# wenet-e2e/wesep

Hardware: AMD Instinct MI355X
Metric: utterances/sec (4 s, 16 kHz, 2-spk) fwd+bwd, pBSRNN (higher is better)
Workload: dtype bf16x3+fp16x2+fp16x1 split products (+fp8 lo terms), fp32 accumulate; 1 GPU; pBSRNN FiLM multi-fuse, 6 repeats, feature_dim 128, fixed 256-d embeddings; fwd + SI-SDR + bwd + per-tensor clip + Adam-L2; bf16x3 (x-projections, projections, d(hcat), BN / mask GEMMs) + fp16x2 (recurrent products of all four recurrence kernels, d(xn)) + fp16x1 (LSTM weight gradients); 2-byte saved gates / d(gates); fp32 accumulate; BPTT kernels: W_hh as fp16 hi + block-scaled FP8 lo; the lo term; rows_per_gpu=32, global_rows=32, samples_per_row=64000, parallelism=dp1

## Files before the change

include/wesep_hip.h:

```cpp
#ifndef WESEP_HIP_H_
#define WESEP_HIP_H_

#ifdef __cplusplus
extern "C" {
#endif

#define WS_ABI_VERSION 20
#define WS_OK 0
#define WS_ERR_INVALID (-1)
#define WS_ERR_LAUNCH (-2)

int ws_abi_version(void);
const char* ws_last_error(void);

#define WS_PROF_LSTM_FWD 0
#define WS_PROF_LSTM_BWD 1
#define WS_PROF_GEMM_NT 2
#define WS_PROF_GEMM_TN 3
#define WS_PROF_NKINDS 4
int ws_prof_enable(int on);
int ws_prof_collect(int kind, double* total_ms, long long* launches);
int ws_debug_dirty_lds(float value, int nblocks, int spins, float* sink, void* stream);
int ws_debug_occupy(int nblocks, int usec, const unsigned* stop, float* sink, void* stream);

// ... 236 lines not shown

typedef struct ws_gemm_b2p_args {
  const float* A;
  const float* Wpack;
  const float* bias;
  const float* R;
  float* C;
  ws_seqmap sm;
  long long ldc;
  int N, K;
  int a_fmt, pad_;
  const unsigned* amax;
  void* a16_out;
} ws_gemm_b2p_args;
int ws_gemm_b2p(const ws_gemm_b2p_args* a, void* stream);

typedef struct ws_gemm_tnb_args {
  const float* G;
  const float* A0;
  const float* A1;
  float* slab;
  float* bslab;
  float* aslab;
  long long slab_stride, bslab_stride, aslab_stride;
  int g_width, g_off, g_cols;
  int a0_width, a0_off, a0_cols, a0_shift;
  int a1_width, a1_off, a1_cols, a1_shift;
  int nblk, L, nsplit, blocks_per_split;
  int g_fmt;
  const unsigned* amax;
  int a_fmt, pad_;
} ws_gemm_tnb_args;
int ws_gemm_tnb(const ws_gemm_tnb_args* a, void* stream);

typedef struct ws_bands {
  const int* band_of_bin;
  const int* band_f0;
  const int* band_bw;
  int nband, nbins;
} ws_bands;
int ws_stft_bandsplit(const float* wav, int R, int T, const ws_bands* b, float* xbs, void* stream);
int ws_stft_bandsplit_len(const float* wav, int R, int T, const int* lengths, const ws_bands* b, float* xbs, void* stream);
int ws_mask_istft_frames(const float* xbs, const float* mask3, int R, int Tf, const ws_bands* b,
                         float* frames, void* stream);
int ws_istft_ola(const float* frames, int R, int Tf, int T, float* wav, void* stream);
int ws_istft_ola_len(const float* frames, int R, int Tf, int T, const int* lengths, float* wav, void* stream);
int ws_mask_istft_bwd(const float* dwav, const float* xbs, const float* mask3, int R, int Tf,
                      int T, const ws_bands* b, float* dmask3, void* stream);

int ws_affine_fwd(const float* z, const float* a, const float* b, float a0, long long rows,
                  int rows_per_r, int N, float* out, void* stream);
int ws_affine_bwd(const float* dz, const float* z_in, const float* a, float a0, long long rows,
                  int rows_per_r, int N, int nsplit, float* dz_in, float* da_slab, float* db_slab,
                  float* da, float* db, unsigned* counter, void* stream);

int ws_sisdr_fwd(const float* est, const float* tgt, int R, int T, float eps, float* rowstat,
                 float* loss, void* stream);
int ws_sisdr_bwd(const float* est, const float* tgt, const float* rowstat, const float* gout,
                 int R, int T, float* dest, void* stream);

typedef struct ws_tensor_ref {
  float* param;
  float* grad;
  float* exp_avg;
  float* exp_avg_sq;
  long long numel;
// ... 233 lines not shown
```

wesep_amd/_lib.py:

```python
import ctypes as C
import os

import numpy as np
import torch

_HERE = os.path.dirname(os.path.abspath(__file__))
LIB_PATH = os.environ.get("WESEP_HIP_LIB") or os.path.join(_HERE, "libwesep_hip.so")

WS_OK = 0
PROF_LSTM_FWD, PROF_LSTM_BWD, PROF_GEMM_NT, PROF_GEMM_TN = 0, 1, 2, 3
LSTM_H = 256
ABI_VERSION = 20
GATES_F32, GATES_H2, GATES_H2S, GATES_H2F = 0, 1, 2, 3
DGATES_EXP = 8


def dgates_scale(amax_bits: int) -> float:
    e = (int(amax_bits) >> 23) & 0xFF
    return 1.0 if e in (0, 255) else 2.0 ** (min(max(DGATES_EXP + 254 - e, 1), 253) - 127)


LSTM_F32_MT1, LSTM_F32_MT2, LSTM_BF16X3, LSTM_BF16X3_BLK, LSTM_BF16X3_BLK16 = 1, 2, 3, 4, 5
LSTM_PACK_FLOATS = 2 * 4 * LSTM_H * LSTM_H

# ... 136 lines not shown
    "ws_pack_w_f16": (_i, [_p, _i, _i, _ll, _i, _i, _p, _p]),
    "ws_pack_w_f16f8": (_i, [_p, _i, _i, _ll, _i, _p, _p]),
    "ws_gemm_nt": (_i, [C.POINTER(GemmNTArgs), _p]),
    "ws_gemm_tn": (_i, [C.POINTER(GemmTNArgs), _p]),
    "ws_reduce_slabs": (_i, [_p, _i, _ll, _ll, _p, _i, _ll, _p]),
    "ws_transpose": (_i, [_p, _i, _i, _ll, _p, _p]),
    "ws_group_stats": (_i, [_p, C.POINTER(GroupsGeom), _f, _p, _p]),
    "ws_group_stats_len": (_i, [_p, C.POINTER(GroupsGeom), _p, _i, _f, _p, _p]),
    "ws_gn_bwd_reduce": (_i, [_p, _p, _p, _p, _p, C.POINTER(GroupsGeom), _p, _p]),
    "ws_gn_bwd_apply": (_i, [_p, _p, _p, _p, _p, _p, _p, C.POINTER(GroupsGeom), _p, _p]),
    "ws_gn_param_grad": (_i, [_p, _p, _p, C.POINTER(GroupsGeom), _i, _p, _p]),
    "ws_gn_bwd_fused": (_i, [_p, _p, _p, _p, _p, C.POINTER(GroupsGeom), _i, _p, _p, _p, _p, _p]),
    "ws_gn_bwd_fused2": (_i, [_p, _p, _p, _p, _p, _p, C.POINTER(GroupsGeom), _i, _p, _p, _p, _p, _p]),
    "ws_gn_bwd_apply_pg": (_i, [_p, _p, _p, _p, _p, _p, C.POINTER(GroupsGeom), _p, _p, _p, _p, _p]),
    "ws_lstm_pack": (_i, [_p, _p, _p, _p, _i, _p]),
    "ws_lstm_fwd": (_i, [C.POINTER(LstmArgs), _p]),
    "ws_lstm_bwd": (_i, [C.POINTER(LstmArgs), _p]),
    "ws_lstm_fwd_cluster": (_i, [C.POINTER(LstmClusterArgs), _p]),
    "ws_lstm_bwd_cluster": (_i, [C.POINTER(LstmClusterArgs), _p]),
    "ws_lstm_fwd_cluster2": (_i, [C.POINTER(LstmCluster2Args), _p]),
    "ws_lstm_pack_pair": (_i, [_p, _p, _p, _p]),
    "ws_lstm_pack_pair_f16": (_i, [_p, _p, _p, _p]),
    "ws_lstm_pack_pair_f8": (_i, [_p, _p, _p, _p]),
    "ws_lstm_pack_pair_f8mx": (_i, [_p, _p, _p, _p]),
    "ws_lstm_pack_bwd_f8": (_i, [_p, _p, _p, _p]),
    "ws_lstm_pack_dx_f8": (_i, [_p, _p, _p]),
    "ws_lstm_bwd_pair": (_i, [C.POINTER(LstmPairArgs), _p]),
    "ws_lstm_cat_ih": (_i, [_p, _p, _p, _p, _p, _p, _i, _p, _p, _p]),
    "ws_pack_w": (_i, [_p, _i, _i, _ll, _i, _i, _p, _p]),
    "ws_gemm_p2b": (_i, [C.POINTER(GemmP2BArgs), _p]),
    "ws_gemm_p2b_len": (_i, [C.POINTER(GemmP2BArgs), _p, _i, _p]),
    "ws_gemm_b2p": (_i, [C.POINTER(GemmB2PArgs), _p]),
    "ws_gemm_tnb": (_i, [C.POINTER(GemmTNBArgs), _p]),
    "ws_stft_bandsplit": (_i, [_p, _i, _i, C.POINTER(Bands), _p, _p]),
    "ws_stft_bandsplit_len": (_i, [_p, _i, _i, _p, C.POINTER(Bands), _p, _p]),
    "ws_mask_istft_frames": (_i, [_p, _p, _i, _i, C.POINTER(Bands), _p, _p]),
    "ws_istft_ola": (_i, [_p, _i, _i, _i, _p, _p]),
    "ws_istft_ola_len": (_i, [_p, _i, _i, _i, _p, _p, _p]),
    "ws_mask_istft_bwd": (_i, [_p, _p, _p, _i, _i, _i, C.POINTER(Bands), _p, _p]),
    "ws_affine_fwd": (_i, [_p, _p, _p, _f, _ll, _i, _i, _p, _p]),
    "ws_affine_bwd": (_i, [_p, _p, _p, _f, _ll, _i, _i, _i, _p, _p, _p, _p, _p, _p, _p]),
    "ws_sisdr_fwd": (_i, [_p, _p, _i, _i, _f, _p, _p, _p]),
    "ws_sisdr_bwd": (_i, [_p, _p, _p, _p, _i, _i, _p, _p]),
    "ws_flat_stats": (_i, [_p, _i, _ll, C.c_float, _i, _p, _p, _p]),
    "ws_prelu_fwd": (_i, [_p, _p, _p, _ll, _i, _i, _p, _p]),
    "ws_prelu_bwd": (_i, [_p, _p, _p, _ll, _p, _p, _i, _p]),
    "ws_dwconv_fwd": (_i, [_p, _p, _p, _p, _p, _p, _i, _i, _i, _i, _i, _i, _p, _p]),
    "ws_dwconv_bwd": (_i, [_p, _p, _p, _p, _p, _p, _i, _i, _i, _i, _i, _i, _p, _i, _i, _p, _p]),
    "ws_dwconv_ex_fwd": (_i, [_p, _p, _p, _p, _p, _p, _i, _i, _i, _i, _i, _i, _i, _p, _p]),
    "ws_dwconv_ex_bwd": (_i, [_p, _p, _p, _p, _p, _p, _i, _i, _i, _i, _i, _i, _i, _p, _i, _i, _p, _p]),
    "ws_chan_sums": (_i, [_p, _p, _p, _i, _i, _i, _i, _i, _p, _p]),
    "ws_norm_ab": (_i, [_p, _p, _i, _i, _ll, _p, _p]),
    "ws_norm_bwd_apply_cl": (_i, [_p, _p, _p, _p, _p, _p, _ll, _i, _i, _p, _p]),
    "ws_maskmul_fwd": (_i, [_p, _ll, _p, _ll, _i, _p, _p]),
    "ws_maskmul_bwd": (_i, [_p, _p, _ll, _p, _ll, _i, _p, _ll, _p, _p]),
    "ws_relu_mask": (_i, [_p, _p, _ll, _p]),
    "ws_ola_fwd": (_i, [_p, _p, _i, _i, _i, _i, _i, _p, _p]),
    "ws_ola_bwd": (_i, [_p, _i, _i, _i, _i, _i, _p, _p]),
    "ws_sum_partial": (_i, [_p, _ll, _p, _i, _p]),
    "ws_bn_stats": (_i, [_p, _ll, _i, C.c_float, C.c_float, _p, _p, _i, _p, _p, _p]),
    "ws_bn_prelu_fwd": (_i, [_p, _p, _p, _p, _p, _p, _ll, _i, _p, _p, _p]),
    "ws_bn_bwd": (_i, [_p, _p, _p, _p, _ll, _i, _i, _p, _p, _p, _p]),
    "ws_maxpool3_fwd": (_i, [_p, _i, _i, _i, _p, _p]),
    "ws_maxpool3_bwd": (_i, [_p, _p, _i, _i, _i, _p, _p]),
    "ws_bcast_rows": (_i, [_p, C.c_float, _i, _ll, _i, _p, _p]),
    "ws_cross_entropy": (_i, [_p, _p, _i, _i, _p, _p, _p]),
# ... 123 lines not shown
```

wesep_amd/blstm_core.py:

```python
import math
import os
from typing import NamedTuple

import numpy as np
import torch

from . import _lib as L
from . import dev

H = L.LSTM_H
G4 = 4 * H
N = 128


def _empty(dev_, *shape):
    return torch.empty(*shape, device=dev_, dtype=torch.float32)


def _reduce_new(slab, nsplit, stride, shape):
    out = _empty(slab.device, *shape)
    dev.reduce_slabs(slab, nsplit, stride, int(np.prod(shape)), out)
    return out


# ... 1 lines not shown
    return int(os.environ.get("WESEP_H2_PROBE", "0"))


_PROBE_SAT = [0, 0.0]


def _probe_round(t, kind, packed=False):
    if kind == "f16":
        t.copy_(t.half().float())
    elif kind == "u16":
        v = t.view(-1, 2, 4, 64 * 128)
        v[:, :, 2].mul_(0.5).add_(0.5)
        v.copy_(torch.floor(v * 65535.0 + 0.5) / 65535.0)
        v[:, :, 2].mul_(2.0).sub_(1.0)
    elif packed and torch.cuda.is_available():
        t.view(torch.int32).bitwise_and_(-65536)
    else:
        t.copy_(t.bfloat16().float())


def tnb_a16() -> bool:
    return os.environ.get("WESEP_TNB_A16", "1") != "0"


def pair_rfmt(gfmt) -> int:
    rf = int(os.environ.get("WESEP_PAIR_RF", "3"))
    if rf not in (0, 1, 2, 3):
        raise ValueError(f"WESEP_PAIR_RF={rf}: 0, 1, 2 or 3")
    return rf if gfmt == L.GATES_H2F else 0


def dxn_fmt(g_fmt) -> int:
    return 3 if g_fmt == 2 and os.environ.get("WESEP_DXN_F8", "1") != "0" else g_fmt


def band_rfmt(gfmt, lmode) -> int:
    rf = int(os.environ.get("WESEP_BAND_RF", "3"))
    if rf not in (0, 2, 3):
        raise ValueError(f"WESEP_BAND_RF={rf}: 0, 2 or 3")
    if rf == 3 and os.environ.get("WESEP_BAND_DX", "0") == "1":
        rf = 2
    return rf if gfmt == L.GATES_H2F and lmode == L.LSTM_BF16X3_BLK else 0


def band_dx(brf, seq, geo) -> bool:
    return (brf == 2 and os.environ.get("WESEP_BAND_DX", "0") == "1" and not seq.nvalid and dev.gn_bwd_fused_ok(geo))


_SIDE_STREAMS = {}


def _side_stream(device):
    key = (device.type, device.index)
    if key not in _SIDE_STREAMS:
        pr = os.environ.get("WESEP_SIDE_PRIORITY")
        _SIDE_STREAMS[key] = torch.cuda.Stream(device=device, priority=int(pr)) if pr else torch.cuda.Stream(device=device)
    return _SIDE_STREAMS[key]


_PENDING = {}


def _pending(device):
    return _PENDING.setdefault((device.type, device.index), [])


# ... 206 lines not shown
            dev.lstm_pack(*W("whh"), pack_f, pack_b, lmode)
            return pack_f, pack_b
        if kind == "hh8":
            pack = _empty(d, L.LSTM_PACK_FLOATS)
            dev.lstm_pack_bwd_f8(*W("whh"), pack)
            return pack
        if kind == "wx8":
            pack = _empty(d, L.LSTM_DX_PACK_FLOATS)
            dev.lstm_pack_dx_f8(W("cat")[0], pack)
            return pack
        if kind in ("hhp", "hhp16"):
            pack = _empty(d, L.LSTM_PACK_FLOATS)
            dev.lstm_pack_pair(*W("whh"), pack, f16=pair_rf if kind == "hhp16" else 0)
            return pack
        if kind in ("fused", "fused16", "fused8"):
            fpack = _empty(d, L.LSTM_FUSED_PACK_FLOATS)
            dev.lstm_pack_fused(wih_f.contiguous(), wih_r.contiguous(), *W("whh"), fpack,
                                hfmt={"fused": 0, "fused16": 1, "fused8": 5}[kind])
            return fpack
        if kind == "wih":
            out = _empty(d, 2 * G4 * N)
            dev.pack_w(W("cat")[0], 2 * G4, N, N, out, order=0)
            return out
        if kind in ("wihT", "wihT16", "wihT8"):
            out = _empty(d, N * 2 * G4)
            dev.pack_w(W("cat")[0], N, 2 * G4, N, out, trans=True, order=1, f16={"wihT": 0, "wihT16": 1, "wihT8": 2}[kind])
            return out
        if kind == "pw":
            return proj_w.contiguous()
        if kind == "proj":
            out = _empty(d, N * 2 * H)
            dev.pack_w(W("pw"), N, 2 * H, 2 * H, out, order=1)
            return out
        if kind == "projT":
            out = _empty(d, 2 * H * N)
            dev.pack_w(W("pw"), 2 * H, N, 2 * H, out, trans=True, order=0)
            return out
        raise KeyError(kind)


class BlstmPlan(NamedTuple):
    nb: int
    lmode: int
    cluster: bool
    fwd: str
    bptt: str
    grad: bool
    gfmt: int
    g_fmt: int
    a16: bool
    pair_rfmt: int
    band_rfmt: int
    band_dx: bool
    a_fmt: int


_WIHT_KIND = {0: "wihT", 1: "wihT", 2: "wihT16", 3: "wihT8"}


def make_plan(seq, device, grad, gn_geo=None, ragged=False) -> BlstmPlan:
    lmode = dev.lstm_blk_mode(seq.nseq)
    cluster = dev.lstm_cluster_ok(seq, device)
    bptt = _bptt_kind(seq, device, cluster)
    gfmt = L.GATES_F32 if bptt == "cluster" else dev.gates_fmt()
    h2 = gfmt != L.GATES_F32
    if ragged:
        fwd = "cluster" if cluster else "stream"
    elif dev.lstm_fuse_ok(seq.nseq, cluster):
        fwd = "fused"
    elif cluster:
        fwd = "cluster2" if h2 and dev.lstm_cluster2_on() else "cluster"
    else:
        fwd = "stream"
    g_fmt = {L.GATES_H2: 1, L.GATES_H2F: 2}.get(gfmt, 0)
    brf = band_rfmt(gfmt, lmode) if grad and bptt == "stream" else 0
    return BlstmPlan(
        nb=dev.bl_num_blocks(seq), lmode=lmode, cluster=cluster, fwd=fwd, bptt=bptt, grad=grad, gfmt=gfmt, g_fmt=g_fmt,
        a16=gfmt == L.GATES_H2F and grad and tnb_a16(), pair_rfmt=pair_rfmt(gfmt) if grad and bptt == "pair" else 0,
        band_rfmt=brf, band_dx=bool(brf) and gn_geo is not None and band_dx(brf, seq, gn_geo), a_fmt=dxn_fmt(g_fmt))


def consume_once(ctx, who):
    if ctx.consumed:
        raise L.WesepHipError(f"{who}: second backward through the same graph (retain_graph / multi-loss loops): "
                              "the blocked path consumes its saved gates in place; run the forward again")
    ctx.consumed = True


def blstm_forward(plan, W, x, seq, res, bias, norm=None, steps=None):
    d = x.device
    norm = norm or {}
    if steps is not None and (plan.fwd in ("fused", "cluster2") or plan.grad):
        raise L.WesepHipError(f"blstm_forward: per-sequence step counts with forward branch '{plan.fwd}', grad={plan.grad}: "
                              "only the branches over precomputed gates know them, and only the forward")
    lens = dict(steps=steps[0], steps_div=steps[1]) if steps is not None else {}
    nb, gfmt, lmode = plan.nb, plan.gfmt, plan.lmode
    h2 = gfmt != L.GATES_F32
    wcat, bcat = W("cat")
    whf, whr = W("whh")
    xn = _empty(d, nb, 32 * N)
    cbuf, hcat = _empty(d, nb, 32 * 2 * H), _empty(d, nb, 32 * 2 * H)
    gates = _empty(d, dev.blh_floats(nb, 2 * G4)) if h2 else _empty(d, nb, 32 * 2 * G4)
    xn16 = _empty(d, dev.blh_floats(nb, N)) if plan.a16 else None
    hcat16 = _empty(d, dev.blh_floats(nb, 2 * H)) if plan.a16 else None
    if plan.fwd == "fused":
        dev.gemm_p2b(A=x, lda=N, sm=seq, Wpack=None, N=0, C_out=None, A_bl=xn, A_bl16=xn16, **norm)
        hf = dev.lstm_fused_hfmt(gfmt)
        dev.lstm_fwd_fused(gates, cbuf, hcat, xn, W("fused8" if hf & 4 else "fused16" if hf else "fused"), bcat, seq, gfmt=gfmt,
                           hfmt=hf)
    elif plan.fwd == "cluster2":
        dev.gemm_p2b(A=x, lda=N, sm=seq, Wpack=None, N=0, C_out=None, A_bl=xn, A_bl16=xn16, **norm)
        tw = dev.lstm_fwd_cluster2(gates, cbuf, hcat, xn, wcat, bcat, whf, whr, seq, dbg=_cluster_dbg())
        pre = dev.fallback_scratch(d, nb * 32 * 2 * G4)
        dev.gemm_p2b(A=x, lda=N, sm=seq, Wpack=W("wih"), N=2 * G4, C_out=pre, bias=bcat, run_if=tw, **norm)
        dev.lstm_fwd(gates, cbuf, hcat, W("hh")[0], seq, lmode, run_if=tw, gfmt=gfmt, gates_in=pre)
        del pre
    else:
        pre = _empty(d, nb, 32 * 2 * G4) if h2 else gates
        xproj = dict(A=x, lda=N, sm=seq, Wpack=W("wih"), N=2 * G4, C_out=pre, bias=bcat, A_bl=xn, A_bl16=xn16, **norm, **lens)
        rec = dict(gfmt=gfmt, gates_in=pre) if h2 else {}
        dev.gemm_p2b(**xproj)
        if _h2_probe() & 768 and not torch.cuda.is_available():
            pre.copy_(pre.half().float() if _h2_probe() & 256 else pre.bfloat16().float())
        if plan.fwd == "cluster":
            tw = dev.lstm_fwd_cluster(gates, cbuf, hcat, whf, whr, seq, dbg=_cluster_dbg(), **rec)
            if not h2:
                dev.gemm_p2b(run_if=tw, **xproj)
            dev.lstm_fwd(gates, cbuf, hcat, W("hh")[0], seq, lmode, run_if=tw, **rec)
        else:
            dev.lstm_fwd(gates, cbuf, hcat, W("hh")[0], seq, lmode, **rec)
        del pre
    out = torch.empty_like(res)
    dev.gemm_b2p(A=hcat, K=2 * H, sm=seq, Wpack=W("proj"), C_out=out, ldc=N, bias=bias, R=res, a16_out=hcat16)
    if _h2_probe() and not h2:
        if _h2_probe() & 1:
            _probe_round(gates, "f16")
        if _h2_probe() & 8:
            _probe_round(gates, "u16")
        if _h2_probe() & 4:
            _probe_round(cbuf, "f16")
    if plan.grad:
        W("projT")
        if not plan.band_dx:
            W(_WIHT_KIND[plan.a_fmt])
        if plan.bptt == "pair":
            W("hhp16" if plan.pair_rfmt else "hhp")
        if (plan.bptt == "stream" and not plan.band_rfmt) or (plan.bptt == "pair" and h2):
            W("hh")
        if plan.bptt == "stream" and plan.band_rfmt:
            W("hh8")
            if plan.band_dx:
                W("wx8")
    return out, (gates, cbuf, hcat, xn16 if plan.a16 else xn, hcat16)


def blstm_bptt(plan, W, gates, cbuf, hcat, dout, seq, release):
    d = dout.device
    nb, gfmt = plan.nb, plan.gfmt
    dh, dout_bl = _empty(d, nb, 32 * 2 * H), _empty(d, nb, 32 * N)
    dxn2 = None
    amax = amax_word(d) if gfmt == L.GATES_H2F else None
    dev.gemm_p2b(A=dout, lda=N, sm=seq, Wpack=W("projT"), N=2 * H, C_out=dh, A_bl=dout_bl, amax=amax)
    if _h2_probe() & 16:
        _probe_round(dh, "bf16")
    ready = mark_wgrads_ready(d) if release else None
    if plan.bptt == "cluster":
        dg = gates
        dev.lstm_bwd_cluster(gates, cbuf, dh, *W("whh"), seq)
    elif gfmt == L.GATES_F32:
        dg = gates
        if plan.bptt == "pair":
            dev.lstm_bwd_pair(gates, cbuf, dh, W("hhp"), seq, dbg=_pair_dbg())
        else:
            dev.lstm_bwd(gates, cbuf, hcat, dh, W("hh")[1], seq, plan.lmode)
    elif plan.bptt == "pair":
        dg = _empty(d, nb, 32 * 2 * G4) if gfmt == L.GATES_H2S else _empty(d, dev.blh_floats(nb, 2 * G4))
        rf = plan.pair_rfmt
        tw = dev.lstm_bwd_pair(gates, cbuf, dh, W("hhp16" if rf else "hhp"), seq, gfmt=gfmt, dgates=dg, repairable=True,
                               dbg=_pair_dbg(), amax=amax, rfmt=rf, dbg_buf=_pair_stamp_buf(d, seq.L))
        dev.lstm_bwd(gates, cbuf, hcat, dh, W("hh")[1], seq, plan.lmode, gfmt=gfmt, dgates=dg, run_if=tw, amax=amax)
    else:
        dg = _empty(d, nb, 32 * 2 * G4) if gfmt == L.GATES_H2S else gates
        brf = plan.band_rfmt
        if plan.band_dx:
            dxn2 = _empty(d, 2, dout.numel() // N, N)
        dev.lstm_bwd(gates, cbuf, hcat, dh, W("hh8") if brf else W("hh")[1], seq, plan.lmode, gfmt=gfmt,
                     dgates=dg if gfmt == L.GATES_H2S else None, amax=amax, rfmt=brf, dxn=dxn2,
                     wxpack=W("wx8") if dxn2 is not None else None)
    if _h2_probe() & 2 and gfmt == L.GATES_F32:
        _probe_round(gates, "bf16", packed=True)
    if _h2_probe() & 32 and gfmt == L.GATES_F32 and not torch.cuda.is_available():
        amax = float(dh.abs().max())
        S = 2.0 ** (10 - math.floor(math.log2(amax))) if amax > 0 and math.isfinite(amax) else 1.0
        sc = gates * S
        _PROBE_SAT[0] += int((sc.abs() > 65504.0).sum())
        _PROBE_SAT[1] = max(_PROBE_SAT[1], float(sc.abs().max()) / 65504.0)
        gates.copy_(sc.clamp(-65504.0, 65504.0).half().float() / S)
    if ready is not None:
        flush_deferred_wgrads(d, ready)
    return dg, dout_bl, amax, dxn2


def weight_grads(gates, xn, hcat, dout_bl, seq, nb, g_fmt=0, amax=None, hcat16=None):
    d = gates.device
    a_fmt = 1 if hcat16 is not None else 0
    if _h2_probe() & 192 and not torch.cuda.is_available() and not a_fmt:
        rnd = (lambda t: t.half().float()) if _h2_probe() & 64 else (lambda t: t.bfloat16().float())
        xn, hcat = rnd(xn), rnd(hcat)
    if os.environ.get("WESEP_PROBE_SKIP_WGRAD") == "1":
        z_ = lambda *s_: torch.zeros(*s_, device=d)
        return [z_(G4, N), z_(G4, H), z_(G4), z_(G4), z_(G4, N), z_(G4, H), z_(G4), z_(G4), z_(N, 2 * H), z_(N)]
    if _h2_probe() & 1024 and not torch.cuda.is_available() and amax is not None:
        S = L.dgates_scale(int(amax.reshape(-1)[0]))
        hcat = hcat.half().float()
        dout_bl = (dout_bl * S).half().float() / S
    ns, bps = dev.tnb_splits(nb, (2 * H) // 128)
    slab, aslab = _empty(d, ns, 2 * H * N), _empty(d, ns, N)
    dev.gemm_tnb(G=hcat, g_width=2 * H, g_off=0, g_cols=2 * H, A0=dout_bl, a0_width=N, a0_off=0, a0_cols=N,
                 nblk=nb, L_=seq.L, slab=slab, nsplit=ns, blocks_per_split=bps, aslab=aslab)
    dproj_w = _reduce_new(slab, ns, 2 * H * N, (2 * H, N)).t().contiguous()
    dproj_b = _reduce_new(aslab, ns, N, (N,))
    ns, bps = dev.tnb_splits(nb, G4 // 128)
    slab, bslab = _empty(d, ns, G4 * (N + H)), _empty(d, ns, G4)
    dwih, dwhh, db = [], [], []
    for di in (0, 1):
        dev.gemm_tnb(G=gates, g_width=2 * G4, g_off=di * G4, g_cols=G4, A0=xn, a0_width=N, a0_off=0,
                     a0_cols=N, A1=hcat16 if a_fmt else hcat, a1_width=2 * H, a1_off=di * H, a1_cols=H,
                     a1_shift=(-1 if di == 0 else 1), nblk=nb, L_=seq.L, slab=slab, nsplit=ns,
                     blocks_per_split=bps, bslab=bslab, g_fmt=g_fmt, amax=amax, a_fmt=a_fmt)
        dw = _reduce_new(slab, ns, G4 * (N + H), (G4, N + H))
        dwih.append(dw[:, :N].contiguous())
        dwhh.append(dw[:, N:].contiguous())
        db.append(_reduce_new(bslab, ns, G4, (G4,)))
    return [dwih[0], dwhh[0], db[0], db[0].clone(), dwih[1], dwhh[1], db[1], db[1].clone(),
            dproj_w, dproj_b]


def blstm_weight_grads(plan, dg, xn, hcat, dout_bl, amax, hcat16, seq, box, order=tuple(range(10))):
    if box is None:
        wg = weight_grads(dg, xn, hcat, dout_bl, seq, plan.nb, plan.g_fmt, amax, hcat16)
        return [wg[i] for i in order]
    prod = torch.cuda.current_stream()

    def job(side):
        wg = weight_grads(dg, xn, hcat, dout_bl, seq, plan.nb, plan.g_fmt, amax, hcat16)
        box.grads = [wg[i] for i in order]
        box.event = torch.cuda.Event()
        box.event.record(side)
        keep_for_side(box, (dg, xn, hcat, dout_bl, amax, hcat16), side, prod)
    defer_wgrad(dg.device, job)
    return [None] * len(order)


def blstm_dxn(plan, W, dg, amax, dxn2, seq, rows):
    if dxn2 is not None:
        return dxn2[0], dxn2[1]
    dxn = _empty(dg.device, rows, N)
    dev.gemm_b2p(A=dg, K=2 * G4, sm=seq, Wpack=W(_WIHT_KIND[plan.a_fmt]), C_out=dxn, ldc=N, a_fmt=plan.a_fmt, amax=amax)
    return dxn, None
```

wesep_amd/csrc/gemm_blk.hip:

```cpp
#include <stdlib.h>

#include <type_traits>

#include "common.h"

typedef __bf16 bf16x8 __attribute__((ext_vector_type(8)));
typedef unsigned int u32x4 __attribute__((ext_vector_type(4)));
typedef unsigned int u32x2 __attribute__((ext_vector_type(2)));
typedef float f32x2 __attribute__((ext_vector_type(2)));
typedef _Float16 f16x8 __attribute__((ext_vector_type(8)));
typedef _Float16 f16x2 __attribute__((ext_vector_type(2)));
typedef int i32x4 __attribute__((ext_vector_type(4)));
typedef int v8i __attribute__((ext_vector_type(8)));
typedef __fp16 h16x2 __attribute__((ext_vector_type(2)));

__device__ __forceinline__ f32x16 mfma32(bf16x8 a, bf16x8 b, f32x16 c) {
  return __builtin_amdgcn_mfma_f32_32x32x16_bf16(a, b, c, 0, 0, 0);
}

__device__ __forceinline__ void split8(const float* v, bf16x8& hi, bf16x8& lo) {
#pragma unroll
  for (int j = 0; j < 8; ++j) {
    hi[j] = (__bf16)v[j];
    lo[j] = (__bf16)(v[j] - (float)hi[j]);
// ... 485 lines not shown
      if (off[k] >= 0) *reinterpret_cast<f32x4*>(p.C + off[k]) = v[k];
    __syncthreads();
  }
}

extern "C" int ws_gemm_b2p(const ws_gemm_b2p_args* a, void* stream) {
  WS_REQUIRE(a && a->A && a->Wpack && a->C, "ws_gemm_b2p: null pointer");
  WS_REQUIRE(a->N == 128, "ws_gemm_b2p: N must be 128 (got %d)", a->N);
  WS_REQUIRE(a->a_fmt >= 0 && a->a_fmt <= 3 && (a->a_fmt < 2 || a->amax), "ws_gemm_b2p: a_fmt %d (2 / 3 need amax)", a->a_fmt);
  WS_REQUIRE(a->a_fmt == 0 || !a->a16_out, "ws_gemm_b2p: a16_out goes with a_fmt 0 (got a_fmt %d)", a->a_fmt);
  WS_REQUIRE(a->K > 0 && a->K % 64 == 0, "ws_gemm_b2p: K %% 64 (K=%d)", a->K);
  WS_REQUIRE(a->ldc >= a->N && a->ldc % 4 == 0, "ws_gemm_b2p: ldc >= N and ldc %% 4 == 0 (16-byte row pieces)");
  WS_REQUIRE(a->sm.nseq > 0 && a->sm.L > 0 && a->sm.sq_div > 0, "ws_gemm_b2p: bad sequence map");
  const int nblk = ((a->sm.nseq + 31) / 32) * a->sm.L;
  hipStream_t s = (hipStream_t)stream;
  ws_prof_begin(WS_PROF_GEMM_NT, s);
  if (a->a_fmt == 3)
    hipLaunchKernelGGL(gemm_b2p_kernel<3>, dim3((nblk + 7) / 8), dim3(512), 0, s, *a);
  else if (a->a_fmt == 2)
    hipLaunchKernelGGL(gemm_b2p_kernel<2>, dim3((nblk + 7) / 8), dim3(512), 0, s, *a);
  else if (a->a_fmt == 1)
    hipLaunchKernelGGL(gemm_b2p_kernel<1>, dim3((nblk + 7) / 8), dim3(512), 0, s, *a);
  else
    hipLaunchKernelGGL(gemm_b2p_kernel<0>, dim3((nblk + 7) / 8), dim3(512), 0, s, *a);
  ws_prof_end(WS_PROF_GEMM_NT, s);
  return ws_check_launch("ws_gemm_b2p");
}

typedef __bf16 bf16x4 __attribute__((ext_vector_type(4)));
#define TB_LD 40

typedef __bf16 bf16x2 __attribute__((ext_vector_type(2)));

template <int TA, bool ASUM>
__global__ __launch_bounds__(512, 2) void gemm_tnb_kernel(const ws_gemm_tnb_args p) {
  constexpr int NCOL = 128 * (1 + TA);
  constexpr int PLANE = NCOL * TB_LD;
  constexpr int NG = (1 + TA) / 2;
  constexpr int TN = TA == 1 ? 1 : TA;
  __shared__ __attribute__((aligned(16))) __bf16 ldsA[2 * PLANE];
  __shared__ __attribute__((aligned(16))) __bf16 ldsB[2 * PLANE];
  const int tid = threadIdx.x, lane = tid & 63, l31 = lane & 31, half = lane >> 5;
  const int w = __builtin_amdgcn_readfirstlane(tid >> 6);
  const int wm = w >> 2, wn = w & 3;
  const int gt = blockIdx.y, split = blockIdx.x;
  const int L = p.L;
  const int b_begin = split * p.blocks_per_split;
  const int b_end = min(p.nblk, b_begin + p.blocks_per_split);

  const float* gbase[NG];
  long long gstride[NG];
  int gshift[NG], gcol[NG];
#pragma unroll
  for (int r = 0; r < NG; ++r) {
    const int g = tid + 512 * r;
    const int part = g >> 8, quad = (g >> 3) & 31, sg = g & 7;
    gcol[r] = part * 128 + 4 * quad;
    if (part == 0) {
      gbase[r] = p.G + (long long)((p.g_off + gt * 128) / 4 + quad) * 128 + sg * 16;
      gstride[r] = 32LL * p.g_width;
      gshift[r] = 0;
    } else {
      const int c0 = (part - 1) * 128;
      const bool s1 = c0 >= p.a0_cols;
      const float* base = s1 ? p.A1 : p.A0;
      const int off = s1 ? p.a1_off + c0 - p.a0_cols : p.a0_off + c0;
      gbase[r] = base + (long long)(off / 4 + quad) * 128 + sg * 16;
      gstride[r] = 32LL * (s1 ? p.a1_width : p.a0_width);
      gshift[r] = s1 ? p.a1_shift : p.a0_shift;
    }
  }
  const int sg = tid & 7;

  f32x4 rq[2][NG][4];
  bool use[2][NG];
  auto load_block = [&](int b, int slot) {
    const int tile = b / L, step = b - tile * L;
#pragma unroll
    for (int r = 0; r < NG; ++r) {
      const int sa = step + gshift[r];
      use[slot][r] = sa >= 0 && sa < L;
      const float* src = gbase[r] + (long long)(use[slot][r] ? b + gshift[r] : b) * gstride[r];
#pragma unroll
      for (int j = 0; j < 4; ++j) rq[slot][r][j] = *reinterpret_cast<const f32x4*>(src + 4 * j);
    }
  };
  float csum[NG][4];
#pragma unroll
  for (int r = 0; r < NG; ++r)
#pragma unroll
    for (int c = 0; c < 4; ++c) csum[r][c] = 0.f;
  auto store_piece = [&](int slot, __bf16* lds, unsigned live, int pc) {
    const int r = pc >> 2, c = pc & 3;
    unsigned e[4];
#pragma unroll
    for (int j = 0; j < 4; ++j) {
      const float f = rq[slot][r][j][c];
      e[j] = __float_as_uint(f);
    }
    if (r > 0) {
      const unsigned m = use[slot][r] ? 0xffffffffu : 0u;
#pragma unroll
      for (int j = 0; j < 4; ++j) e[j] &= m;
    }
    if (r == 0 || ASUM) {
      const bf16x2 ones = __builtin_bit_cast(bf16x2, live);
#pragma unroll
      for (int j = 0; j < 4; ++j)
        csum[r][c] = __builtin_amdgcn_fdot2_f32_bf16(__builtin_bit_cast(bf16x2, e[j]), ones, csum[r][c], false);
    }
    uint2 hi, lo;
    hi.x = __builtin_amdgcn_perm(e[1], e[0], WS_SEL_HI16);
    hi.y = __builtin_amdgcn_perm(e[3], e[2], WS_SEL_HI16);
    lo.x = __builtin_amdgcn_perm(e[1], e[0], WS_SEL_LO16);
    lo.y = __builtin_amdgcn_perm(e[3], e[2], WS_SEL_LO16);
    const int o = (gcol[r] + c) * TB_LD + 4 * sg;
    *reinterpret_cast<uint2*>(lds + o) = hi;
    *reinterpret_cast<uint2*>(lds + PLANE + o) = lo;
  };
  auto store_block = [&](int slot, __bf16* lds, unsigned live) {
#pragma unroll
    for (int pc = 0; pc < 4 * NG; ++pc) store_piece(slot, lds, live, pc);
  };

  f32x16 acc[2][TN];
#pragma unroll
  for (int e = 0; e < 2; ++e)
#pragma unroll
    for (int f = 0; f < TN; ++f)
#pragma unroll
      for (int r = 0; r < 16; ++r) acc[e][f][r] = 0.f;
// ... 351 lines not shown
    for (int f = 0; f < TN; ++f) {
      const int ac_ = wn * 32 * TN + f * 32 + l31;
      if (ac_ < ncols) {
#pragma unroll
        for (int r = 0; r < 16; ++r) {
          const int grow = gt * 128 + wm * 64 + e * 32 + (r & 3) + 8 * (r >> 2) + 4 * half;
          out[(long long)grow * ncols + ac_] = GFMT >= 2 ? acc[e][f][r] * inv_out : acc[e][f][r];
        }
      }
    }
#pragma unroll
  for (int c = 0; c < 4; ++c) {
    float t = gsum[c];
    t += __shfl_xor(t, 1, 64);
    t += __shfl_xor(t, 2, 64);
    t += __shfl_xor(t, 4, 64);
    t += __shfl_xor(t, 8, 64);
    if (p.bslab && sp == 0) p.bslab[(long long)split * p.bslab_stride + gt * 128 + 4 * qg + c] = GFMT >= 2 ? t * inv_s : t;
  }
  if (ASUM && gt == 0 && p.aslab) {
#pragma unroll
    for (int r = 0; r < 2; ++r)
#pragma unroll
      for (int c = 0; c < 4; ++c) {
        float t = asum[r][c];
        t += __shfl_xor(t, 1, 64);
        t += __shfl_xor(t, 2, 64);
        t += __shfl_xor(t, 4, 64);
        if (r == 1) t += __shfl_xor(t, 8, 64);
        const bool first = r == 0 ? (tid & 7) == 0 : (tid & 15) == 0;
        if (first) p.aslab[(long long)split * p.aslab_stride + acol[r] - 128 + c] = t;
      }
  }
}

extern "C" int ws_gemm_tnb(const ws_gemm_tnb_args* a, void* stream) {
  WS_REQUIRE(a && a->G && a->A0 && a->slab, "ws_gemm_tnb: null pointer");
  WS_REQUIRE(a->g_cols > 0 && a->g_cols % 128 == 0 && a->g_off % 4 == 0 && a->g_width % 4 == 0,
             "ws_gemm_tnb: G column range");
  WS_REQUIRE(a->a0_cols > 0 && a->a0_cols % 128 == 0 && a->a0_off % 4 == 0 && a->a0_width % 4 == 0,
             "ws_gemm_tnb: A0 column range");
  WS_REQUIRE(a->a1_cols == 0 || (a->A1 && a->a1_cols % 128 == 0 && a->a1_off % 4 == 0 && a->a1_width % 4 == 0),
             "ws_gemm_tnb: A1 column range");
  const int ta = (a->a0_cols + a->a1_cols) / 128;
  WS_REQUIRE(ta == 1 || ta == 3, "ws_gemm_tnb: A columns must total 128 or 384 (got %d)", ta * 128);
  WS_REQUIRE(a->a0_shift == 0, "ws_gemm_tnb: only A1 can be shifted (a0_shift = %d)", a->a0_shift);
  WS_REQUIRE(a->g_fmt == 0 || ((a->g_fmt == 1 || a->g_fmt == 2) && ta == 3),
             "ws_gemm_tnb: g_fmt 1 / 2 (2-byte G) are built for 384 A columns");
  WS_REQUIRE(a->g_fmt != 2 || a->amax, "ws_gemm_tnb: g_fmt = 2 (scaled fp16 G) needs amax");
  WS_REQUIRE(a->a_fmt == 0 || (a->a_fmt == 1 && a->g_fmt == 2 && !a->aslab && ta == 3),
             "ws_gemm_tnb: a_fmt = 1 (fp16 A operands) is built for g_fmt = 2, 384 A columns, no aslab");
  WS_REQUIRE(a->nblk > 0 && a->L > 0 && a->nblk % a->L == 0 && a->nsplit > 0 && a->blocks_per_split > 0 &&
                 (long long)a->nsplit * a->blocks_per_split >= a->nblk,
             "ws_gemm_tnb: bad block split");
  hipStream_t s = (hipStream_t)stream;
  dim3 grid(a->nsplit, a->g_cols / 128), block(512);
  ws_prof_begin(WS_PROF_GEMM_TN, s);
  static const int gdepth = [] { const char* e = getenv("WS_TNB_GDEPTH"); return e && atoi(e) == 2 ? 2 : 4; }();
  const char* f16env = getenv("WS_TNB_F16");
  const bool f16mm = !(f16env && atoi(f16env) == 0);
  if (a->a_fmt == 1)
    hipLaunchKernelGGL((gemm_tnb16_kernel<false, 3, 4, 1>), grid, block, 0, s, *a);
  else if (a->g_fmt == 2 && f16mm && a->aslab)
    hipLaunchKernelGGL((gemm_tnb16_kernel<true, 3, 4>), grid, block, 0, s, *a);
  else if (a->g_fmt == 2 && f16mm)
    hipLaunchKernelGGL((gemm_tnb16_kernel<false, 3, 4>), grid, block, 0, s, *a);
// ... 22 lines not shown
```

wesep_amd/csrc/lstm.hip:

```cpp
#include "common.h"

#define LH WS_LSTM_H
#define LG (4 * LH)
#define HL_LD 68
#define DG_LD 260

__device__ __forceinline__ f32x4 mfma16(float a, float b, f32x4 c) {
  return __builtin_amdgcn_mfma_f32_16x16x4f32(a, b, c, 0, 0, 0);
}

__device__ __forceinline__ float fast_sigmoid(float x) {
  return __builtin_amdgcn_rcpf(1.f + __expf(-x));
}
__device__ __forceinline__ float fast_tanh(float x) {
  const float ax = fabsf(x);
  const float e = __expf(-2.f * ax);
  const float t = (1.f - e) * __builtin_amdgcn_rcpf(1.f + e);
  return copysignf(t, x);
}

__global__ void lstm_pack_kernel(const float* __restrict__ whh_f, const float* __restrict__ whh_r,
                                 float* __restrict__ pf, float* __restrict__ pb) {
  const int total = 2 * LG * LH;
  for (int idx = blockIdx.x * blockDim.x + threadIdx.x; idx < total; idx += gridDim.x * blockDim.x) {
// ... 316 lines not shown
      f32x4 a[MT];
#pragma unroll
      for (int mt = 0; mt < MT; ++mt)
        a[mt] = *reinterpret_cast<const f32x4*>(arow + mt * (64 * DG_LD) + 4 * ks4);
#pragma unroll
      for (int q = 0; q < 4; ++q)
#pragma unroll
        for (int s = 0; s < 2; ++s)
#pragma unroll
          for (int mt = 0; mt < MT; ++mt) dh[mt][s] = mfma16(a[mt][q], bcur[s][q], dh[mt][s]);
      bcur[0] = bnxt[0];
      bcur[1] = bnxt[1];
    }
    __syncthreads();
  }
}

static int lstm_check(const ws_lstm_args* a, bool bwd, const char* who) {
  WS_REQUIRE(a && a->gates && a->cbuf && a->hcat && a->wpack, "%s: null pointer", who);
  WS_REQUIRE(!bwd || a->dhcat, "%s: null dhcat", who);
  WS_REQUIRE(a->nseq > 0 && a->L > 0 && a->sq_div > 0, "%s: bad nseq/L/sq_div", who);
  WS_REQUIRE((a->mode & 255) >= WS_LSTM_F32_MT1 && (a->mode & 255) <= WS_LSTM_BF16X3_BLK16, "%s: bad mode %d", who,
             a->mode);
  WS_REQUIRE(!a->run_if || (!bwd && (a->mode & 255) >= WS_LSTM_BF16X3) || (bwd && (a->mode & 255) >= WS_LSTM_BF16X3_BLK),
             "%s: run_if is honoured by the split-bf16 forward kernels and the blocked-layout BPTT kernels only", who);
  WS_REQUIRE(a->gfmt >= WS_GATES_F32 && a->gfmt <= WS_GATES_H2F, "%s: bad gfmt %d", who, a->gfmt);
  WS_REQUIRE(a->gfmt != WS_GATES_H2F || !bwd || a->amax, "%s: WS_GATES_H2F needs amax", who);
  WS_REQUIRE(a->gfmt == WS_GATES_F32 || (a->mode & 255) >= WS_LSTM_BF16X3_BLK,
             "%s: gfmt %d is a format of the blocked-layout modes", who, a->gfmt);
  WS_REQUIRE(a->gfmt == WS_GATES_F32 || bwd || a->gates_in, "%s: gfmt %d needs gates_in (the fp32 pre-activations)", who,
             a->gfmt);
  WS_REQUIRE(a->gfmt != WS_GATES_H2S || !bwd || a->dgates, "%s: WS_GATES_H2S needs dgates", who);
  WS_REQUIRE(a->gfmt == WS_GATES_F32 || ((a->mode >> 8) & 7) == 0, "%s: probe builds are WS_GATES_F32 only", who);
  WS_REQUIRE(a->rfmt == 0 || ((a->rfmt == 2 || a->rfmt == 3) && bwd && a->mode == WS_LSTM_BF16X3_BLK && a->gfmt == WS_GATES_H2F),
             "%s: rfmt %d (2 / 3 = fp16 recurrence on fp16 + FP8 weights, 3: the lo term on the FP8 MFMA: ws_lstm_bwd, "
             "WS_LSTM_BF16X3_BLK, WS_GATES_H2F only)", who, a->rfmt);
  WS_REQUIRE(!a->dxn || (bwd && a->rfmt == 2 && a->wxpack && a->dxn_dir_stride > 0 && a->dxn_dir_stride < (1ll << 29) && !a->run_if),
             "%s: dxn (d(xn) inside the BPTT, ABI v19) needs rfmt 2, wxpack (ws_lstm_pack_dx_f8), 0 < dxn_dir_stride < 2^29 floats "
             "(32-bit store offsets) and no run_if", who);
  return WS_OK;
}

extern "C" int ws_lstm_fwd(const ws_lstm_args* a, void* stream) {
  int rc = lstm_check(a, false, "ws_lstm_fwd");
  if (rc != WS_OK) return rc;
  hipStream_t s = (hipStream_t)stream;
  const int per = 16 * a->mode;
  dim3 grid((a->nseq + per - 1) / per, 2), block(512);
  const bool timed = a->run_if == nullptr;
  if (timed) ws_prof_begin(WS_PROF_LSTM_FWD, s);
  if ((a->mode & 255) == WS_LSTM_BF16X3_BLK16)
    ws_launch_lstm_fwd_s16(a, s);
  else if ((a->mode & 255) >= WS_LSTM_BF16X3)
    ws_launch_lstm_fwd_bf16(a, s);
  else if (a->mode == WS_LSTM_F32_MT1)
    hipLaunchKernelGGL((lstm_fwd_kernel<1>), grid, block, 0, s, *a);
  else
    hipLaunchKernelGGL((lstm_fwd_kernel<2>), grid, block, 0, s, *a);
  if (timed) ws_prof_end(WS_PROF_LSTM_FWD, s);
  return ws_check_launch("ws_lstm_fwd");
}

extern "C" int ws_lstm_bwd(const ws_lstm_args* a, void* stream) {
  int rc = lstm_check(a, true, "ws_lstm_bwd");
  if (rc != WS_OK) return rc;
  hipStream_t s = (hipStream_t)stream;
  const int per = 16 * a->mode;
  dim3 grid((a->nseq + per - 1) / per, 2), block(512);
  const bool timed = a->run_if == nullptr;
// ... 13 lines not shown
```

wesep_amd/csrc/lstm_bf16.hip:

```cpp
#include <stdlib.h>

#include "lstm_bf16_common.h"

__global__ void lstm_pack_bf16_kernel(const float* __restrict__ whh_f, const float* __restrict__ whh_r,
                                      __bf16* __restrict__ pf, __bf16* __restrict__ pb) {
  const int total = 2 * LG * LH;
  for (int idx = blockIdx.x * blockDim.x + threadIdx.x; idx < total; idx += gridDim.x * blockDim.x) {
    {
      int r = idx;
      const int j = r & 7; r >>= 3;
      const int lane = r & 63; r >>= 6;
      const int g = r & 3; r >>= 2;
      const int ks = r & 15; r >>= 4;
      const int w = r & 7; r >>= 3;
      const int d = r;
      const float* W = d ? whh_r : whh_f;
      const int row = g * 256 + 32 * w + (lane & 31);
      const int k = 16 * ks + 8 * (lane >> 5) + j;
      const float v = W[row * LH + k];
      const __bf16 hi = (__bf16)v;
      const long long unit = ((((long long)(d * 8 + w) * 16 + ks) * 4 + g) * 2) * 64 + lane;
      pf[unit * 8 + j] = hi;
      pf[(unit + 64) * 8 + j] = (__bf16)(v - (float)hi);
    }
// ... 82 lines not shown
    v0[i] = 256.f * W[row * 128 + u];
    v1[i] = 256.f * W[(row + 1) * 128 + u];
    m = fmaxf(m, fmaxf(fabsf(v0[i]), fabsf(v1[i])));
  }
#pragma unroll
  for (int o = 32; o > 0; o >>= 1) m = fmaxf(m, __shfl_xor(m, o));
  if ((tid & 63) == 0) red[tid >> 6] = m;
  __syncthreads();
  m = red[0];
#pragma unroll
  for (int i = 1; i < 8; ++i) m = fmaxf(m, red[i]);
  const int eb = (int)((__builtin_bit_cast(unsigned, m) >> 23) & 0xffu);
  const float S = (eb > 19 && eb < 255) ? __builtin_bit_cast(float, (unsigned)(eb - 19) << 23) : 1.f;
  char* ob = px + (long long)(d * 8 + w) * WS_DX_REGION;
  if (tid == 0) reinterpret_cast<float*>(ob + 48 * 1024)[grp] = S;
#pragma unroll
  for (int i = 0; i < 2; ++i) {
    const int pi = tid + 512 * i, j2 = pi & 3, lane = (pi >> 2) & 63, f = pi >> 8;
    const _Float16 h0 = (_Float16)v0[i], h1 = (_Float16)v1[i];
    typedef _Float16 f16x2 __attribute__((ext_vector_type(2)));
    typedef short s16x2 __attribute__((ext_vector_type(2)));
    char* cb = ob + (2 * grp + (f >> 1)) * 3072;
    *reinterpret_cast<f16x2*>(cb + (f & 1) * 1024 + lane * 16 + j2 * 4) = f16x2{h0, h1};
    const s16x2 c = __builtin_amdgcn_cvt_scalef32_pk_fp8_f32(s16x2{0, 0}, v0[i] - (float)h0, v1[i] - (float)h1, S, false);
    *reinterpret_cast<short*>(cb + 2048 + (f & 1) * 512 + lane * 8 + j2 * 2) = c[0];
  }
}

int ws_launch_lstm_pack_dx_f8(const float* wcat, float* pack, hipStream_t s) {
  hipLaunchKernelGGL(lstm_pack_dx_f8_kernel, dim3(128), dim3(512), 0, s, wcat, reinterpret_cast<char*>(pack));
  return 0;
}

template <bool BLK, int DBG, int GF = 0>
__global__ __launch_bounds__(512, 2) void lstm_fwd_bf16_kernel(const ws_lstm_args p) {
  __shared__ __attribute__((aligned(16))) __bf16 hl[2][2][SQ * HROW];
  __shared__ __attribute__((aligned(16))) float cl[SQ * (LH + 4)];
  if (p.run_if && *p.run_if == 0u) return;
  const int d = blockIdx.y;
  const int tid = threadIdx.x, lane = tid & 63, l31 = lane & 31, half = lane >> 5;
  const int w = __builtin_amdgcn_readfirstlane(tid >> 6);
  const int L = p.L;

  {
    uint32_t* z = reinterpret_cast<uint32_t*>(&hl[0][0][0]);
    for (int i = tid; i < 2 * SQ * HROW / 2; i += 512) z[i] = 0u;
  }
  const int ss = min((int)blockIdx.x * SQ + l31, p.nseq - 1);
  const long long rowbase =
      BLK ? 0 : (long long)(ss / p.sq_div) * p.sq_s1 + (long long)(ss % p.sq_div) * p.sq_s2;
  const int ubase = 32 * w + 4 * half;
  const int glane = ((d * 256 + 8 * w + half) * 32 + l31) * 16;
  const int clane = ((d * 64 + 8 * w + half) * 32 + l31) * 16;
  auto goff = [&](int t, int g, int j) -> long long {
    return ((rowbase + (long long)t * p.step_rows) * 2 + d) * LG + g * 256 + ubase + 8 * j;
  };
  auto coff = [&](int t, int j) -> long long {
    return (rowbase + (long long)t * p.step_rows) * (2 * LH) + d * LH + ubase + 8 * j;
  };
  const float* gsrc = GF ? p.gates_in : p.gates;
  auto grs = [&](int t) { return mkrsrc(gsrc + (long long)(blockIdx.x * L + t) * (SQ * 2 * LG), SQ * 2 * LG * 4); };
  auto hrs = [&](int t) { return mkrsrc(p.gates + (long long)(blockIdx.x * L + t) * (SQ * LG), SQ * 2 * LG * 2); };
  auto crs = [&](float* b, int t) { return mkrsrc(b + (long long)(blockIdx.x * L + t) * (SQ * 2 * LH), SQ * 2 * LH * 4); };
  auto ld_gate = [&](int t, int g, int j) -> f32x4 {
    if constexpr (BLK) return bld(grs(t), glane, (g * 64 + 2 * j) * 512);
    else return *reinterpret_cast<const f32x4*>(p.gates + goff(t, g, j));
  };
  auto st_gate = [&](const f32x4& v, int t, int g, int j) {
    if constexpr (GF != 0) bst8(g == 2 ? enc_u16x4<true>(v) : enc_u16x4<false>(v), hrs(t), glane >> 1, (g * 64 + 2 * j) * 256);
    else if constexpr (BLK) bst(v, grs(t), glane, (g * 64 + 2 * j) * 512);
    else *reinterpret_cast<f32x4*>(p.gates + goff(t, g, j)) = v;
  };
  auto st_ch = [&](const f32x4& v, float* b, int t, int j) {
    if constexpr (BLK) bst(v, crs(b, t), clane, 2 * j * 512);
    else *reinterpret_cast<f32x4*>(b + coff(t, j)) = v;
  };

  float* cme = &cl[l31 * (LH + 4) + ubase];
#pragma unroll
  for (int j = 0; j < 4; ++j) *reinterpret_cast<f32x4*>(cme + 8 * j) = f32x4{0.f, 0.f, 0.f, 0.f};

  const __amdgpu_buffer_rsrc_t wrs = __builtin_amdgcn_make_buffer_rsrc(
      const_cast<float*>(p.wpack) + (long long)(d * 8 + w) * (16 * 8 * 64 * 4), 0, 16 * 8 * 1024, 0x00020000);
  const int wlane = lane * 16;
  bf16x8 wr[2][8];
#pragma unroll
  for (int s = 0; s < 2; ++s)
#pragma unroll
    for (int f = 0; f < 8; ++f) wr[s][f] = wload(wrs, wlane + (f & 3) * 1024, s * 8192 + (f >> 2) * 4096);

  f32x4 xg[4][4];
  {
    const int t0 = d == 0 ? 0 : L - 1;
#pragma unroll
    for (int gi = 0; gi < 4; ++gi)
#pragma unroll
      for (int j = 0; j < 4; ++j) xg[gi][j] = ld_gate(t0, gi, j);
  }
  __syncthreads();

  for (int step = 0; step < L; ++step) {
    const int t = d == 0 ? step : L - 1 - step;
    const int cur = step & 1;
    int zo = 0;
    asm volatile("" : "+s"(zo));
    const __bf16* hhi = &hl[cur][0][l31 * HROW + 8 * half];
    const __bf16* hlo = &hl[cur][1][l31 * HROW + 8 * half];
    f32x16 acc[4];
#pragma unroll
// ... 43 lines not shown
    for (int j = 0; j < 4; ++j) {
      f32x4 pre[4];
#pragma unroll
      for (int g = 0; g < 4; ++g)
#pragma unroll
        for (int r = 0; r < 4; ++r) pre[g][r] = acc[g][4 * j + r];
      f32x4 vi, vf, vg, vo, vc, vh;
      const f32x4 cold = *reinterpret_cast<const f32x4*>(cme + 8 * j);
#pragma unroll
      for (int r = 0; r < 4; ++r) {
        const float ig = fsig(pre[0][r]);
        const float fg = fsig(pre[1][r]);
        const float gg = ftanh(pre[2][r]);
        const float og = fsig(pre[3][r]);
        const float cn = fg * cold[r] + ig * gg;
        vi[r] = ig;
        vf[r] = fg;
        vg[r] = gg;
        vo[r] = og;
        vc[r] = cn;
        vh[r] = og * ftanh(cn);
      }
      bf16x4 h_hi, h_lo;
      split4(vh, h_hi, h_lo);
      *reinterpret_cast<bf16x4*>(nhi + 8 * j) = h_hi;
      *reinterpret_cast<bf16x4*>(nlo + 8 * j) = h_lo;
      *reinterpret_cast<f32x4*>(cme + 8 * j) = vc;
      if (!(DBG & 1) || step == L - 1) {
        st_gate(vi, t, 0, j);
        st_gate(vf, t, 1, j);
        st_gate(vg, t, 2, j);
        st_gate(vo, t, 3, j);
        st_ch(vc, p.cbuf, t, j);
        if constexpr (BLK) st_ch(pack_hl4(h_hi, h_lo), p.hcat, t, j);
        else st_ch(vh, p.hcat, t, j);
      }
      __builtin_amdgcn_sched_barrier(0);
    }
    __syncthreads();
  }
}

template <bool BLK, int DBG, int GF = 0, int RF = 0, bool DX = false>
__global__ __launch_bounds__(512, 2) void lstm_bwd_bf16_kernel(const ws_lstm_args p) {
  static_assert(RF == 0 || (BLK && GF == WS_GATES_H2F), "the fp16 recurrence takes the scaled-fp16 d(gates) of WS_GATES_H2F");
  static_assert(!DX || RF == 2, "d(xn) in the BPTT rides on the fp16 d(gates) image of rfmt 2");
  __shared__ __attribute__((aligned(16))) __bf16 dgl[RF ? 1 : 2][SQ * DROW];
  __shared__ __attribute__((aligned(16))) f32x4 xred[DX ? 8 * 2 * 64 : 1];
  if (p.run_if && *p.run_if == 0u) return;
  const int d = blockIdx.y, bx = blockIdx.x;
  const int tid = threadIdx.x, lane = tid & 63, l31 = lane & 31, half = lane >> 5;
  const int w = __builtin_amdgcn_readfirstlane(tid >> 6);
  const int L = p.L;
  const int ss = min(bx * SQ + l31, p.nseq - 1);
  const long long rowbase =
      BLK ? 0 : (long long)(ss / p.sq_div) * p.sq_s1 + (long long)(ss % p.sq_div) * p.sq_s2;
  const int ubase = 32 * w + 4 * half;
  const int glane = ((d * 256 + 8 * w + half) * 32 + l31) * 16;
  const int clane = ((d * 64 + 8 * w + half) * 32 + l31) * 16;
  auto goff = [&](int t, int g, int j) -> long long {
    return ((rowbase + (long long)t * p.step_rows) * 2 + d) * LG + g * 256 + ubase + 8 * j;
  };
  auto coff = [&](int t, int j) -> long long {
    return (rowbase + (long long)t * p.step_rows) * (2 * LH) + d * LH + ubase + 8 * j;
  };
  float* gdst = GF == WS_GATES_H2S ? p.dgates : p.gates;
  auto grs = [&](int t) { return mkrsrc(gdst + (long long)(bx * L + t) * (SQ * 2 * LG), SQ * 2 * LG * 4); };
  auto hrs = [&](int t) { return mkrsrc(p.gates + (long long)(bx * L + t) * (SQ * LG), SQ * 2 * LG * 2); };
// ... 269 lines not shown
    if constexpr (DX) {
      const float us = (1.f / 256.f) / dS;
      const unsigned trow = (unsigned)t * (unsigned)p.step_rows * 512u;
#pragma unroll
      for (int i = 0; i < 2; ++i) {
        const f32x4 o = xred[((w ^ 4) * 2 + i) * 64 + lane];
        __builtin_amdgcn_raw_buffer_store_b128(__builtin_bit_cast(u32x4, (keep[i] + o) * us), xors, xoff + trow + 32 * i, 0, 0);
      }
    }
  }
}

#define WS_DBG_DISPATCH(KERNEL)                                                          \
  if ((a->mode & 255) == WS_LSTM_BF16X3_BLK && a->gfmt == WS_GATES_H2) {                 \
    hipLaunchKernelGGL((KERNEL<true, 0, WS_GATES_H2>), grid, block, 0, s, *a);           \
  } else if ((a->mode & 255) == WS_LSTM_BF16X3_BLK && a->gfmt == WS_GATES_H2S) {         \
    hipLaunchKernelGGL((KERNEL<true, 0, WS_GATES_H2S>), grid, block, 0, s, *a);          \
  } else if ((a->mode & 255) == WS_LSTM_BF16X3_BLK && a->gfmt == WS_GATES_H2F) {         \
    hipLaunchKernelGGL((KERNEL<true, 0, WS_GATES_H2F>), grid, block, 0, s, *a);          \
  } else if ((a->mode & 255) == WS_LSTM_BF16X3_BLK) {                                    \
    switch ((a->mode >> 8) & 7) {                                                        \
      case 0: hipLaunchKernelGGL((KERNEL<true, 0>), grid, block, 0, s, *a); break;       \
      case 1: hipLaunchKernelGGL((KERNEL<true, 1>), grid, block, 0, s, *a); break;       \
      case 2: hipLaunchKernelGGL((KERNEL<true, 2>), grid, block, 0, s, *a); break;       \
      case 4: hipLaunchKernelGGL((KERNEL<true, 4>), grid, block, 0, s, *a); break;       \
      default: hipLaunchKernelGGL((KERNEL<true, 7>), grid, block, 0, s, *a); break;      \
    }                                                                                    \
  } else {                                                                               \
    hipLaunchKernelGGL((KERNEL<false, 0>), grid, block, 0, s, *a);                       \
  }

int ws_launch_lstm_fwd_bf16(const ws_lstm_args* a, hipStream_t s) {
  dim3 grid((a->nseq + SQ - 1) / SQ, 2), block(512);
  WS_DBG_DISPATCH(lstm_fwd_bf16_kernel)
  return 0;
}

int ws_launch_lstm_bwd_bf16(const ws_lstm_args* a, hipStream_t s) {
  dim3 grid((a->nseq + SQ - 1) / SQ, 2), block(512);
  if (a->rfmt == 2 && a->dxn) {
    hipLaunchKernelGGL((lstm_bwd_bf16_kernel<true, 0, WS_GATES_H2F, 2, true>), grid, block, 0, s, *a);
    return 0;
  }
  if (a->rfmt == 2) {
    hipLaunchKernelGGL((lstm_bwd_bf16_kernel<true, 0, WS_GATES_H2F, 2>), grid, block, 0, s, *a);
    return 0;
  }
  if (a->rfmt == 3) {
    hipLaunchKernelGGL((lstm_bwd_bf16_kernel<true, 0, WS_GATES_H2F, 3>), grid, block, 0, s, *a);
    return 0;
  }
  WS_DBG_DISPATCH(lstm_bwd_bf16_kernel)
  return 0;
}
```

wesep_amd/csrc/lstm_bf16_common.h:

```cpp
#pragma once
#include "common.h"

typedef __bf16 bf16x8 __attribute__((ext_vector_type(8)));
typedef __bf16 bf16x4 __attribute__((ext_vector_type(4)));

#define LH WS_LSTM_H
#define LG (4 * LH)
#define SQ 32
#define HROW 264
#define DROW 1032

typedef unsigned int u32x4 __attribute__((ext_vector_type(4)));

__device__ __forceinline__ bf16x8 wload(__amdgpu_buffer_rsrc_t rsrc, int voff, int soff) {
  return __builtin_bit_cast(bf16x8, __builtin_amdgcn_raw_buffer_load_b128(rsrc, voff, soff, 0));
}

__device__ __forceinline__ __amdgpu_buffer_rsrc_t mkrsrc(const float* base, unsigned bytes) {
  return __builtin_amdgcn_make_buffer_rsrc(const_cast<float*>(base), 0, bytes, 0x00020000);
}
#ifndef WS_STREAM_AUX
#define WS_STREAM_AUX 2
#endif
__device__ __forceinline__ f32x4 bld(__amdgpu_buffer_rsrc_t r, int voff, int soff) {
// ... 65 lines not shown

__device__ __forceinline__ u32x2 bld8(__amdgpu_buffer_rsrc_t r, int voff, int soff) {
  return __builtin_bit_cast(u32x2, __builtin_amdgcn_raw_buffer_load_b64(r, voff, soff, WS_STREAM_AUX));
}
__device__ __forceinline__ void bst8(const u32x2& v, __amdgpu_buffer_rsrc_t r, int voff, int soff) {
  __builtin_amdgcn_raw_buffer_store_b64(v, r, voff + soff, 0, WS_STREAM_AUX);
}
template <bool TANH>
__device__ __forceinline__ u32x2 enc_u16x4(const f32x4& v) {
  const float s = TANH ? WS_U16_TANH : WS_U16_SIG, o = TANH ? WS_U16_TANH + 0.5f : 0.5f;
  unsigned u[4];
#pragma unroll
  for (int j = 0; j < 4; ++j) u[j] = (unsigned)__builtin_fmaf(v[j], s, o);
  return u32x2{u[0] | (u[1] << 16), u[2] | (u[3] << 16)};
}
template <bool TANH>
__device__ __forceinline__ f32x4 dec_u16x4(const u32x2& c) {
  const float s = TANH ? 1.f / WS_U16_TANH : 1.f / WS_U16_SIG, o = TANH ? -1.f : 0.f;
  f32x4 v;
  v[0] = __builtin_fmaf((float)(c[0] & 0xffffu), s, o);
  v[1] = __builtin_fmaf((float)(c[0] >> 16), s, o);
  v[2] = __builtin_fmaf((float)(c[1] & 0xffffu), s, o);
  v[3] = __builtin_fmaf((float)(c[1] >> 16), s, o);
  return v;
}
__device__ __forceinline__ u32x2 bf16x4_bits(const bf16x4& v) { return __builtin_bit_cast(u32x2, v); }
typedef _Float16 f16x4 __attribute__((ext_vector_type(4)));
__device__ __forceinline__ u32x2 enc_f16x4(const f32x4& vs) {
  f16x4 h;
#pragma unroll
  for (int j = 0; j < 4; ++j) h[j] = (_Float16)vs[j];
  return __builtin_bit_cast(u32x2, h);
}
template <int GF>
__device__ __forceinline__ u32x2 enc_dgates(const f32x4& v, const bf16x4& hi) {
  if constexpr (GF == WS_GATES_H2F) return enc_f16x4(v);
  else return bf16x4_bits(hi);
}
template <int GF>
__device__ __forceinline__ float dh_in(float dh, float rec, float S) {
  if constexpr (GF == WS_GATES_H2F) return __builtin_fmaf(dh, S, rec);
  else return dh + rec;
}

template <int GF> struct gate_cell { typedef f32x4 type; };
template <> struct gate_cell<WS_GATES_H2> { typedef u32x2 type; };
template <> struct gate_cell<WS_GATES_H2S> { typedef u32x2 type; };
template <> struct gate_cell<WS_GATES_H2F> { typedef u32x2 type; };
template <bool TANH> __device__ __forceinline__ f32x4 gate_val(const f32x4& c) { return c; }
template <bool TANH> __device__ __forceinline__ f32x4 gate_val(const u32x2& c) { return dec_u16x4<TANH>(c); }
```

wesep_amd/csrc/lstm_bf16_s16.hip:

```cpp
#include "lstm_bf16_common.h"

#define S16 16

__device__ __forceinline__ f32x4 mfma16(bf16x8 a, bf16x8 b, f32x4 c) {
  return __builtin_amdgcn_mfma_f32_16x16x32_bf16(a, b, c, 0, 0, 0);
}

__global__ void lstm_pack_s16_kernel(const float* __restrict__ whh_f, const float* __restrict__ whh_r,
                                     __bf16* __restrict__ pf, __bf16* __restrict__ pb) {
  const int total = 2 * LG * LH;
  for (int idx = blockIdx.x * blockDim.x + threadIdx.x; idx < total; idx += gridDim.x * blockDim.x) {
    {
      int r = idx;
      const int j = r & 7; r >>= 3;
      const int lane = r & 63; r >>= 6;
      const int tile = r & 7; r >>= 3;
      const int ks = r & 7; r >>= 3;
      const int w = r & 7; r >>= 3;
      const int d = r;
      const float* W = d ? whh_r : whh_f;
      const int row = (tile >> 1) * 256 + 32 * w + 16 * (tile & 1) + (lane & 15);
      const int k = 32 * ks + 8 * (lane >> 4) + j;
      const float v = W[row * LH + k];
      const __bf16 hi = (__bf16)v;
      const long long unit = ((((long long)(d * 8 + w) * 8 + ks) * 8 + tile) * 2) * 64 + lane;
      pf[unit * 8 + j] = hi;
      pf[(unit + 64) * 8 + j] = (__bf16)(v - (float)hi);
    }
    {
      int r = idx;
      const int j = r & 7; r >>= 3;
      const int lane = r & 63; r >>= 6;
      const int tu = r & 1; r >>= 1;
      const int ks = r & 31; r >>= 5;
      const int w = r & 7; r >>= 3;
      const int d = r;
      const float* W = d ? whh_r : whh_f;
      const int row = 32 * ks + 8 * (lane >> 4) + j;
      const int u = 32 * w + 16 * tu + (lane & 15);
      const float v = W[row * LH + u];
      const __bf16 hi = (__bf16)v;
      const long long unit = ((((long long)(d * 8 + w) * 32 + ks) * 2 + tu) * 2) * 64 + lane;
      pb[unit * 8 + j] = hi;
      pb[(unit + 64) * 8 + j] = (__bf16)(v - (float)hi);
    }
  }
}

int ws_launch_lstm_pack_s16(const float* whh_f, const float* whh_r, float* pack_fwd, float* pack_bwd,
                            hipStream_t s) {
  hipLaunchKernelGGL(lstm_pack_s16_kernel, dim3(512), dim3(256), 0, s, whh_f, whh_r,
                     reinterpret_cast<__bf16*>(pack_fwd), reinterpret_cast<__bf16*>(pack_bwd));
  return 0;
}

template <int GF>
__global__ __launch_bounds__(512, 2) void lstm_fwd_s16_kernel(const ws_lstm_args p) {
  __shared__ __attribute__((aligned(16))) __bf16 hl[2][2][S16 * HROW];
  __shared__ __attribute__((aligned(16))) float cl[S16 * (LH + 4)];
  if (p.run_if && *p.run_if == 0u) return;
  const int d = blockIdx.y;
  const int tile = blockIdx.x >> 1, hb = blockIdx.x & 1;
  const int tid = threadIdx.x, lane = tid & 63, n = lane & 15, mq = lane >> 4;
  const int w = __builtin_amdgcn_readfirstlane(tid >> 6);
  const int L = p.L;
  {
    uint32_t* z = reinterpret_cast<uint32_t*>(&hl[0][0][0]);
    for (int i = tid; i < 2 * S16 * HROW / 2; i += 512) z[i] = 0u;
  }
  const int glane = ((d * 256 + 8 * w + mq) * 32 + 16 * hb + n) * 16;
  const int clane = ((d * 64 + 8 * w + mq) * 32 + 16 * hb + n) * 16;
  const float* gsrc = GF ? p.gates_in : p.gates;
  auto grs = [&](int t) { return mkrsrc(gsrc + (long long)(tile * L + t) * (SQ * 2 * LG), SQ * 2 * LG * 4); };
  auto hrs = [&](int t) { return mkrsrc(p.gates + (long long)(tile * L + t) * (SQ * LG), SQ * 2 * LG * 2); };
  auto crs = [&](float* b, int t) { return mkrsrc(b + (long long)(tile * L + t) * (SQ * 2 * LH), SQ * 2 * LH * 4); };
  auto ld_gate = [&](int t, int g, int tu) -> f32x4 { return bld(grs(t), glane, (g * 64 + 4 * tu) * 512); };
  auto st_gate = [&](const f32x4& v, int t, int g, int tu) {
    if constexpr (GF != 0) bst8(g == 2 ? enc_u16x4<true>(v) : enc_u16x4<false>(v), hrs(t), glane >> 1, (g * 64 + 4 * tu) * 256);
    else bst(v, grs(t), glane, (g * 64 + 4 * tu) * 512);
  };
  auto st_ch = [&](const f32x4& v, float* b, int t, int tu) { bst(v, crs(b, t), clane, 4 * tu * 512); };

  const int ubase = 32 * w + 4 * mq;
  float* cme = &cl[n * (LH + 4) + ubase];
#pragma unroll
  for (int tu = 0; tu < 2; ++tu) *reinterpret_cast<f32x4*>(cme + 16 * tu) = f32x4{0.f, 0.f, 0.f, 0.f};

  const __amdgpu_buffer_rsrc_t wrs = __builtin_amdgcn_make_buffer_rsrc(
      const_cast<float*>(p.wpack) + (long long)(d * 8 + w) * (8 * 16 * 64 * 4), 0, 8 * 16 * 1024, 0x00020000);
  const int wlane = lane * 16;
  bf16x8 wr[2][16];
#pragma unroll
  for (int s = 0; s < 2; ++s)
#pragma unroll
    for (int f = 0; f < 16; ++f) wr[s][f] = wload(wrs, wlane + (f & 3) * 1024, s * 16384 + (f >> 2) * 4096);

  f32x4 xg[4][2];
  {
    const int t0 = d == 0 ? 0 : L - 1;
#pragma unroll
    for (int g = 0; g < 4; ++g)
#pragma unroll
      for (int tu = 0; tu < 2; ++tu) xg[g][tu] = ld_gate(t0, g, tu);
  }
  __syncthreads();

  for (int step = 0; step < L; ++step) {
    const int t = d == 0 ? step : L - 1 - step;
    const int cur = step & 1;
    int zo = 0;
    asm volatile("" : "+s"(zo));
    const __bf16* hhi = &hl[cur][0][n * HROW + 8 * mq];
    const __bf16* hlo = &hl[cur][1][n * HROW + 8 * mq];
    f32x4 acc[4][2];
// ... 40 lines not shown
#pragma unroll
      for (int g = 0; g < 4; ++g) xg[g][tu] = ld_gate(tn, g, tu);
    __builtin_amdgcn_sched_barrier(0);
    __bf16* nhi = &hl[cur ^ 1][0][n * HROW + ubase];
    __bf16* nlo = &hl[cur ^ 1][1][n * HROW + ubase];
#pragma unroll
    for (int tu = 0; tu < 2; ++tu) {
      f32x4 vi, vf, vg, vo, vc, vh;
      const f32x4 cold = *reinterpret_cast<const f32x4*>(cme + 16 * tu);
#pragma unroll
      for (int r = 0; r < 4; ++r) {
        const float ig = fsig(acc[0][tu][r]);
        const float fg = fsig(acc[1][tu][r]);
        const float gg = ftanh(acc[2][tu][r]);
        const float og = fsig(acc[3][tu][r]);
        const float cn = fg * cold[r] + ig * gg;
        vi[r] = ig;
        vf[r] = fg;
        vg[r] = gg;
        vo[r] = og;
        vc[r] = cn;
        vh[r] = og * ftanh(cn);
      }
      bf16x4 h_hi, h_lo;
      split4(vh, h_hi, h_lo);
      *reinterpret_cast<bf16x4*>(nhi + 16 * tu) = h_hi;
      *reinterpret_cast<bf16x4*>(nlo + 16 * tu) = h_lo;
      *reinterpret_cast<f32x4*>(cme + 16 * tu) = vc;
      st_gate(vi, t, 0, tu);
      st_gate(vf, t, 1, tu);
      st_gate(vg, t, 2, tu);
      st_gate(vo, t, 3, tu);
      st_ch(vc, p.cbuf, t, tu);
      st_ch(pack_hl4(h_hi, h_lo), p.hcat, t, tu);
      __builtin_amdgcn_sched_barrier(0);
    }
    __syncthreads();
  }
}


#ifndef S16_DBG
#define S16_DBG 0
#endif
template <int GF>
__global__ __launch_bounds__(512, 2) void lstm_bwd_s16_kernel(const ws_lstm_args p) {
  __shared__ __attribute__((aligned(16))) __bf16 dgl[2][S16 * DROW];
  if (p.run_if && *p.run_if == 0u) return;
  const int d = blockIdx.y;
  const int tile = blockIdx.x >> 1, hb = blockIdx.x & 1;
  const int tid = threadIdx.x, lane = tid & 63, n = lane & 15, mq = lane >> 4;
  const int w = __builtin_amdgcn_readfirstlane(tid >> 6);
  const int L = p.L;
  const int glane = ((d * 256 + 8 * w + mq) * 32 + 16 * hb + n) * 16;
  const int clane = ((d * 64 + 8 * w + mq) * 32 + 16 * hb + n) * 16;
  float* gdst = GF == WS_GATES_H2S ? p.dgates : p.gates;
  auto grs = [&](int t) { return mkrsrc(gdst + (long long)(tile * L + t) * (SQ * 2 * LG), SQ * 2 * LG * 4); };
  auto hrs = [&](int t) { return mkrsrc(p.gates + (long long)(tile * L + t) * (SQ * LG), SQ * 2 * LG * 2); };
  constexpr bool G2 = GF == WS_GATES_H2 || GF == WS_GATES_H2F;
  float* hdst = (G2 && p.dgates) ? p.dgates : p.gates;
  auto ors = [&](int t) { return mkrsrc(hdst + (long long)(tile * L + t) * (SQ * LG), SQ * 2 * LG * 2); };
  const float dS = GF == WS_GATES_H2F ? ws_dgates_scale(*p.amax) : 1.f;
  auto crs = [&](const float* b, int t) { return mkrsrc(b + (long long)(tile * L + t) * (SQ * 2 * LH), SQ * 2 * LH * 4); };
  typedef typename gate_cell<GF>::type gcell;
  auto ld_gate = [&](int t, int g, int tu) -> gcell {
    if constexpr (GF != 0) return bld8(hrs(t), glane >> 1, (g * 64 + 4 * tu) * 256);
    else return bld(grs(t), glane, (g * 64 + 4 * tu) * 512);
// ... 89 lines not shown
      for (int q = 0; q < 4; ++q) {
        const int ks = 4 * ch + q;
        const bf16x8 bh = *reinterpret_cast<const bf16x8*>(bhi + 32 * ks);
        const bf16x8 bl = *reinterpret_cast<const bf16x8*>(blo + 32 * ks);
#pragma unroll
        for (int tu = 0; tu < 2; ++tu) {
          const int f = (q * 2 + tu) * 2;
          if (ks == 0)
            acc[tu] = mfma16(wr[s][f], bh, zero4v);
          else
            acc[tu] = mfma16(wr[s][f], bh, acc[tu]);
        }
#pragma unroll
        for (int tu = 0; tu < 2; ++tu) acc[tu] = mfma16(wr[s][(q * 2 + tu) * 2 + 1], bh, acc[tu]);
#pragma unroll
        for (int tu = 0; tu < 2; ++tu) acc[tu] = mfma16(wr[s][(q * 2 + tu) * 2], bl, acc[tu]);
      }
      const int cn = (ch + 2) & 7;
      if (!(S16_DBG & 4)) {
#pragma unroll
      for (int f = 0; f < 16; ++f)
        wr[s][f] = wload(wrs, wlane + (f & 3) * 1024, zo + cn * 16384 + (f >> 2) * 4096);
      }
      __builtin_amdgcn_sched_barrier(0);
    }
    dhr[0] = acc[0];
    dhr[1] = acc[1];
    __syncthreads();
  }
}

int ws_launch_lstm_fwd_s16(const ws_lstm_args* a, hipStream_t s) {
  dim3 grid(2 * ((a->nseq + SQ - 1) / SQ), 2), block(512);
  if (a->gfmt) hipLaunchKernelGGL(lstm_fwd_s16_kernel<WS_GATES_H2>, grid, block, 0, s, *a);
  else hipLaunchKernelGGL(lstm_fwd_s16_kernel<0>, grid, block, 0, s, *a);
  return 0;
}

int ws_launch_lstm_bwd_s16(const ws_lstm_args* a, hipStream_t s) {
  dim3 grid(2 * ((a->nseq + SQ - 1) / SQ), 2), block(512);
  if (a->gfmt == WS_GATES_H2) hipLaunchKernelGGL(lstm_bwd_s16_kernel<WS_GATES_H2>, grid, block, 0, s, *a);
  else if (a->gfmt == WS_GATES_H2S) hipLaunchKernelGGL(lstm_bwd_s16_kernel<WS_GATES_H2S>, grid, block, 0, s, *a);
  else if (a->gfmt == WS_GATES_H2F) hipLaunchKernelGGL(lstm_bwd_s16_kernel<WS_GATES_H2F>, grid, block, 0, s, *a);
  else hipLaunchKernelGGL(lstm_bwd_s16_kernel<0>, grid, block, 0, s, *a);
  return 0;
}
```

wesep_amd/csrc/lstm_cluster2.hip:

```cpp
#include "lstm_bf16_common.h"

typedef __attribute__((address_space(1))) unsigned gu32;
#define SC1 16
#define C2_SEQ 64
#define C2_SPIN_LIMIT (1u << 15)
#define C2_TAGS 0x40004000u

__device__ __forceinline__ void split8h(const f32x4& a, const f32x4& b, f16x8& hi, f16x8& lo) {
  const float v[8] = {a[0], a[1], a[2], a[3], b[0], b[1], b[2], b[3]};
#pragma unroll
  for (int j = 0; j < 8; ++j) {
    const float s = 256.f * v[j];
    hi[j] = (_Float16)s;
    lo[j] = (_Float16)(s - (float)hi[j]);
  }
}

__device__ __forceinline__ void split8b(const f32x4& a, const f32x4& b, bf16x8& hi, bf16x8& lo) {
  const float v[8] = {a[0], a[1], a[2], a[3], b[0], b[1], b[2], b[3]};
#pragma unroll
  for (int j = 0; j < 8; ++j) {
    const float s = 256.f * v[j];
    hi[j] = (__bf16)s;
    lo[j] = (__bf16)(s - (float)hi[j]);
// ... 86 lines not shown
      __builtin_amdgcn_sched_barrier(0);
    }
  } else {
    const float* wr = (d ? p.whh_r : p.whh_f) + (long long)wrow * LH + 8 * half;
#pragma unroll
    for (int ks = 0; ks < 16; ++ks)
      split8h(*reinterpret_cast<const f32x4*>(wr + 16 * ks), *reinterpret_cast<const f32x4*>(wr + 16 * ks + 4), wh[ks], wl[ks]);
  }
  {
    const float* xr = p.wcat + ((long long)d * LG + wrow) * 128 + 8 * half;
#pragma unroll
    for (int q = 0; q < 4; ++q) {
      const int ks = 4 * st + q;
      bf16x8 hi, lo;
      split8b(*reinterpret_cast<const f32x4*>(xr + 16 * ks), *reinterpret_cast<const f32x4*>(xr + 16 * ks + 4), hi, lo);
      wih[((uo * 2 + 0) * 8 + ks) * 64 + lane] = hi;
      wih[((uo * 2 + 1) * 8 + ks) * 64 + lane] = lo;
    }
  }
  if (tid < 128)
    reinterpret_cast<float*>(bias_l)[tid] = 256.f * p.bcat[(long long)d * LG + (tid >> 5) * LH + 32 * j + (tid & 31)];
  {
    uint32_t* z = reinterpret_cast<uint32_t*>(hl);
    for (int i = tid; i < C2_SEQ * HROW / 2; i += 512) z[i] = 0u;
    if (tid == 0) dead_s = 0;
  }
  const int mt = tid & 255;
  const int m_uo = (mt >> 6) & 3, m_n = mt & 31, m_half = (mt >> 5) & 1;
  const int gvo = ((d * 256 + 8 * j + 2 * m_uo + m_half) * 32 + m_n) * 16;
  const int cvo = ((d * 64 + 8 * j + 2 * m_uo + m_half) * 32 + m_n) * 16;
  const int gts = (int)(L * gblk * 4), cts = (int)(L * cblk * 4);
  auto hrs = [&](int t) { return mkrsrc(p.gates + ((long long)2 * cc * L + t) * (gblk / 2), 0x7fffffffu); };
  auto crs = [&](float* b, int t) { return mkrsrc(b + ((long long)2 * cc * L + t) * cblk, 0x7fffffffu); };
  const char* xbase = reinterpret_cast<const char*>(p.xn);
  auto xld = [&](int t, int q) -> f32x4 {
    const long long blk = (long long)(2 * cc + st) * L + t;
    return bld(mkrsrc(reinterpret_cast<const float*>(xbase + blk * 16384), 16384), (mt + 256 * q) * 16, 0);
  };
  const __amdgpu_buffer_rsrc_t xrs = __builtin_amdgcn_make_buffer_rsrc(
      reinterpret_cast<char*>(p.xchg) + (long long)c * (2 * 8 * 4096), 0, 2 * 8 * 4096, 0x00020000);
  const int mycell = ((w * 32 + n) * 2 + half) * 8;
  unsigned* tword = p.tword;

  auto step_time = [&](int s) { return d == 0 ? s : L - 1 - s; };
  f32x16 acc0;
  auto xpart = [&]() {
#pragma unroll
    for (int q = 0; q < 4; ++q) {
      const f32x4 b4 = bias_l[q * 8 + 2 * uo + half];
      acc0[4 * q] = b4[0], acc0[4 * q + 1] = b4[1], acc0[4 * q + 2] = b4[2], acc0[4 * q + 3] = b4[3];
    }
    const f32x4* xc = xb + st * 1024 + n;
    const bf16x8* wa = &wih[(uo * 2) * 8 * 64 + lane];
#pragma unroll
    for (int ks = 0; ks < 8; ++ks) {
      bf16x4 h0, l0, h1, l1;
      unpack_hl4(xc[(4 * ks + 2 * half) * 32], h0, l0);
      unpack_hl4(xc[(4 * ks + 2 * half + 1) * 32], h1, l1);
      const bf16x8 bh = __builtin_shufflevector(h0, h1, 0, 1, 2, 3, 4, 5, 6, 7);
      const bf16x8 bl = __builtin_shufflevector(l0, l1, 0, 1, 2, 3, 4, 5, 6, 7);
      acc0 = mfma32(wa[ks * 64], bh, acc0);
      acc0 = mfma32(wa[(8 + ks) * 64], bh, acc0);
      acc0 = mfma32(wa[ks * 64], bl, acc0);
    }
  };

  f32x4 c4 = {0.f, 0.f, 0.f, 0.f};
  f32x4 xreg[4];
#pragma unroll
  for (int q = 0; q < 4; ++q) xb[st * 1024 + mt + 256 * q] = xld(step_time(0), q);
  __syncthreads();
  xpart();
#pragma unroll
  for (int q = 0; q < 4; ++q) xreg[q] = xld(step_time(min(1, L - 1)), q);
  __syncthreads();

  auto hbm_out = [&](int tprev) {
#pragma unroll
    for (int e = 0; e < 2; ++e) {
      const int ct = mt + 256 * e;
#pragma unroll
      for (int g2 = 0; g2 < 2; ++g2) {
        const u32x4 pr = __builtin_bit_cast(u32x4, outl[g2][ct]);
        bst8(u32x2{pr[0], pr[1]}, hrs(tprev), (gvo + e * gts) >> 1, (2 * g2) * 64 * 256);
        bst8(u32x2{pr[2], pr[3]}, hrs(tprev), (gvo + e * gts) >> 1, (2 * g2 + 1) * 64 * 256);
      }
      bst(e == 0 ? c4 : outc[mt], crs(p.cbuf, tprev), cvo + e * cts, 0);
      bst(outl[2][ct], crs(p.hcat, tprev), cvo + e * cts, 0);
    }
  };

  for (int step = 0; step < L; ++step) {
    const int par = step & 1;
    const unsigned tag = ((step >> 1) & 1) ? C2_TAGS : 0u;
    C2TS(0);
#pragma unroll
    for (int q = 0; q < 4; ++q) xb[st * 1024 + mt + 256 * q] = xreg[q];
    {
      const int t2 = step_time(min(step + 2, L - 1));
#pragma unroll
      for (int q = 0; q < 4; ++q) xreg[q] = xld(t2, q);
    }
    C2TS(7);
    {
      const _Float16* hb = &hl[(st * 32 + n) * HROW + 8 * half];
      v8i b8;
#pragma unroll
      for (int ks = 0; ks < 16; ++ks) {
        const f16x8 b = *reinterpret_cast<const f16x8*>(hb + 16 * ks);
        acc0 = mfma16h(wh[ks], b, acc0);
        if constexpr (F8) {
          typedef _Float16 f16x2 __attribute__((ext_vector_type(2)));
          typedef short s16x2 __attribute__((ext_vector_type(2)));
#pragma unroll
          for (int i = 0; i < 2; ++i) {
            s16x2 c = {0, 0};
            c = __builtin_amdgcn_cvt_scalef32_pk_fp8_f16(c, f16x2{b[4 * i], b[4 * i + 1]}, 1.f, false);
            c = __builtin_amdgcn_cvt_scalef32_pk_fp8_f16(c, f16x2{b[4 * i + 2], b[4 * i + 3]}, 1.f, true);
            b8[2 * (ks & 3) + i] = __builtin_bit_cast(int, c);
          }
          if ((ks & 3) == 3) acc0 = __builtin_amdgcn_mfma_scale_f32_32x32x64_f8f6f4(w8[ks >> 2], b8, acc0, 0, 0, 0, sA, 0, 127);
// ... 1 lines not shown
          acc0 = mfma16h(wl[ks], b, acc0);
        }
      }
    }
    if (xrole && step > 0) hbm_out(step_time(step - 1));
    C2TS(1);
    __syncthreads();
    C2TS(2);
    {
      f32x4 vi, vf, vg, vo, vh;
#pragma unroll
      for (int r = 0; r < 4; ++r) {
        const float ig = c2_sig256(acc0[r]);
        const float fg = c2_sig256(acc0[4 + r]);
        const float gg = c2_tanh256(acc0[8 + r]);
        const float og = c2_sig256(acc0[12 + r]);
        const float cn = fg * c4[r] + ig * gg;
        c4[r] = cn;
        vi[r] = ig, vf[r] = fg, vg[r] = gg, vo[r] = og;
        vh[r] = og * ftanh(cn);
      }
      const bool dead = dead_s != 0;
      if (dead) vh = f32x4{__builtin_nanf(""), __builtin_nanf(""), __builtin_nanf(""), __builtin_nanf("")};
      u32x2 hc = enc_f16x4(vh);
      hc[0] = (hc[0] & ~C2_TAGS) | tag;
      hc[1] = (hc[1] & ~C2_TAGS) | tag;
      if (!(p.dbg & 4)) __builtin_amdgcn_raw_buffer_store_b64(hc, xrs, mycell + (par * 8 + j) * 4096, 0, SC1);
      const u32x2 ei = enc_u16x4<false>(vi), ef = enc_u16x4<false>(vf), eg = enc_u16x4<true>(vg), eo = enc_u16x4<false>(vo);
      outl[0][tid] = __builtin_bit_cast(f32x4, u32x4{ei[0], ei[1], ef[0], ef[1]});
      outl[1][tid] = __builtin_bit_cast(f32x4, u32x4{eg[0], eg[1], eo[0], eo[1]});
      if (!xrole) outc[mt] = c4;
      bf16x4 hi, lo;
      split4(vh, hi, lo);
      outl[2][tid] = pack_hl4(hi, lo);
    }
    C2TS(3);
    xpart();
    C2TS(4);
    if (xrole) {
      u32x4 pv[8];
      unsigned spins = 0;
      const bool force = FORCE && step == 2 && c == 0 && j == 0;
      bool dead = dead_s != 0;
      while (true) {
        asm volatile("" ::: "memory");
        bool ok = true;
#pragma unroll
        for (int jj = 0; jj < 8; ++jj) {
          pv[jj] = __builtin_amdgcn_raw_buffer_load_b128(xrs, mt * 16, ((par * 8 + jj) * 256) * 16, SC1);
        }
#pragma unroll
        for (int jj = 0; jj < 8; ++jj) {
          const unsigned bad = ((pv[jj][0] ^ tag) | (pv[jj][1] ^ tag) | (pv[jj][2] ^ tag) | (pv[jj][3] ^ tag)) & C2_TAGS;
          ok = ok && bad == 0u;
        }
        if ((ok && !force) || dead || (p.dbg & 1)) break;
        if (force || ++spins > C2_SPIN_LIMIT) {
          cluster2_timed_out(tword, p.status, &dead_s);
          dead = true;
          break;
        }
        __builtin_amdgcn_s_sleep(1);
      }
      C2TS(5);
      _Float16* hrow = &hl[(((mt >> 7) & 1) * 32 + (mt & 31)) * HROW + 8 * ((mt >> 5) & 3)];
#pragma unroll
      for (int jj = 0; jj < 8; ++jj) {
        u32x4 v = pv[jj];
        v[0] &= ~C2_TAGS, v[1] &= ~C2_TAGS, v[2] &= ~C2_TAGS, v[3] &= ~C2_TAGS;
        *reinterpret_cast<u32x4*>(hrow + 32 * jj) = v;
      }
      C2TS(6);
    }
    __syncthreads();
  }
  if (xrole) hbm_out(step_time(L - 1));
}

extern "C" int ws_lstm_fwd_cluster2(const ws_lstm_cluster2_args* a, void* stream) {
  WS_REQUIRE(a && a->gates && a->cbuf && a->hcat && a->xn && a->wcat && a->bcat && a->whh_f && a->whh_r && a->xchg &&
                 a->tword,
             "ws_lstm_fwd_cluster2: null pointer");
  WS_REQUIRE(a->nseq > 0 && a->nseq % 64 == 0 && a->L > 0, "ws_lstm_fwd_cluster2: nseq must be a multiple of 64");
  const int ncl = a->nseq / 32, nwg = ncl * 8;
  int dev = 0, cus = 0;
  (void)hipGetDevice(&dev);
  (void)hipDeviceGetAttribute(&cus, hipDeviceAttributeMultiprocessorCount, dev);
  WS_REQUIRE(nwg <= cus, "ws_lstm_fwd_cluster2: %d workgroups must be co-resident but the device has %d CUs", nwg, cus);
  const int grid = 64 * ((ncl + 7) / 8);
  hipStream_t s = (hipStream_t)stream;
  hipError_t e = hipMemsetAsync(a->xchg, 0x40, (size_t)ncl * (2 * 8 * 4096), s);
  WS_REQUIRE(e == hipSuccess, "ws_lstm_fwd_cluster2: hipMemsetAsync failed");
  e = hipMemsetAsync(a->tword, 0, sizeof(unsigned), s);
  WS_REQUIRE(e == hipSuccess, "ws_lstm_fwd_cluster2: hipMemsetAsync failed");
  ws_prof_begin(WS_PROF_LSTM_FWD, s);
  WS_REQUIRE(a->rfmt == 0 || a->rfmt == 1, "ws_lstm_fwd_cluster2: rfmt %d (0: fp16 hi / lo of W_hh; 1: the lo term on the FP8 MFMA)", a->rfmt);
  if (a->rfmt == 1) {
    if (a->dbg & 2048) hipLaunchKernelGGL((lstm_fwd_cluster2_kernel<false, true, true>), dim3(grid), dim3(512), 0, s, *a);
    else if (a->dbg & 8) hipLaunchKernelGGL((lstm_fwd_cluster2_kernel<true, false, true>), dim3(grid), dim3(512), 0, s, *a);
    else hipLaunchKernelGGL((lstm_fwd_cluster2_kernel<false, false, true>), dim3(grid), dim3(512), 0, s, *a);
  } else if (a->dbg & 2048) hipLaunchKernelGGL((lstm_fwd_cluster2_kernel<false, true>), dim3(grid), dim3(512), 0, s, *a);
  else if (a->dbg & 8) hipLaunchKernelGGL((lstm_fwd_cluster2_kernel<true>), dim3(grid), dim3(512), 0, s, *a);
  else hipLaunchKernelGGL((lstm_fwd_cluster2_kernel<false>), dim3(grid), dim3(512), 0, s, *a);
  ws_prof_end(WS_PROF_LSTM_FWD, s);
  return ws_check_launch("ws_lstm_fwd_cluster2");
}
```

wesep_amd/csrc/lstm_fused.hip:

```cpp
#include <stdlib.h>

#include "lstm_bf16_common.h"

#define XROW 136
#define FKS 24
#define H8ROW 272

template <bool H16>
__global__ void lstm_pack_fused_kernel(const float* __restrict__ wih_f, const float* __restrict__ wih_r,
                                       const float* __restrict__ whh_f, const float* __restrict__ whh_r,
                                       __bf16* __restrict__ pf) {
  const int total = 2 * 8 * FKS * 4 * 64 * 8;
  for (int idx = blockIdx.x * blockDim.x + threadIdx.x; idx < total; idx += gridDim.x * blockDim.x) {
    int r = idx;
    const int j = r & 7; r >>= 3;
    const int lane = r & 63; r >>= 6;
    const int g = r & 3; r >>= 2;
    const int ks = r % FKS; r /= FKS;
    const int w = r & 7; r >>= 3;
    const int d = r;
    const int row = g * 256 + 32 * w + (lane & 31);
    float v;
    if (ks < 8) {
      const float* W = d ? wih_r : wih_f;
// ... 75 lines not shown
  for (int j = 0; j < 32; ++j) {
    const float s = 256.f * W[(j >> 4) * 32 + (j & 15)];
    res[j] = s - (float)(_Float16)s;
    mx = fmaxf(mx, fabsf(res[j]));
  }
#pragma unroll
  for (int o = 32; o >= 1; o >>= 1) mx = fmaxf(mx, __shfl_xor(mx, o));
  int E = 0;
  if (mx > 0.f) E = ((__float_as_int(mx) >> 23) & 255) - 127 - 7;
  E = max(E, -126);
  const float inv = __int_as_float((127 - E) << 23);
  unsigned char* reg = pk + (long long)(d * 8 + w) * F8_REGION;
  unsigned int* o = reinterpret_cast<unsigned int*>(reg + F8_HPART + q * F8_KSTEP + 4096 + lane * 16);
#pragma unroll
  for (int j = 0; j < 32; j += 4) {
    int v = 0;
    v = __builtin_amdgcn_cvt_pk_fp8_f32(res[j] * inv, res[j + 1] * inv, v, false);
    v = __builtin_amdgcn_cvt_pk_fp8_f32(res[j + 2] * inv, res[j + 3] * inv, v, true);
    o[(j >> 4) * 256 + ((j & 15) >> 2)] = (unsigned int)v;
  }
  if (lane == 0) reg[F8_SCALES + q] = (unsigned char)(127 + E);
}

extern "C" int ws_lstm_pack_fused_h8(const float* wih_f, const float* wih_r, const float* whh_f, const float* whh_r,
                                     float* pack, void* stream) {
  WS_REQUIRE(wih_f && wih_r && whh_f && whh_r && pack, "ws_lstm_pack_fused_h8: null pointer");
  static_assert(2 * 8 * F8_REGION <= WS_LSTM_FUSED_PACK_FLOATS * 4, "the F8 stream fits the pack of the other formats");
  unsigned char* pk = reinterpret_cast<unsigned char*>(pack);
  hipLaunchKernelGGL(lstm_pack_fused_h8_hi_kernel, dim3(512), dim3(256), 0, (hipStream_t)stream, wih_f, wih_r, whh_f, whh_r, pk);
  hipLaunchKernelGGL(lstm_pack_fused_h8_lo_kernel, dim3(2 * 8 * 16), dim3(64), 0, (hipStream_t)stream, whh_f, whh_r, pk);
  return ws_check_launch("ws_lstm_pack_fused_h8");
}

template <int GF, bool H16 = false, bool F8 = false>
__global__ __launch_bounds__(512, 1) void lstm_fwd_fused_kernel(const ws_lstm_fused_args p) {
  static_assert(!F8 || H16, "the FP8 lo term belongs to the fp16-h kernel");
  __shared__ __attribute__((aligned(16))) __bf16 hl[2][2][SQ * HROW];
  __shared__ __attribute__((aligned(16))) __bf16 xl[2][2][SQ * XROW];
  __shared__ __attribute__((aligned(16))) float cl[SQ * (LH + 4)];
  const int d = blockIdx.y;
  const int tid = threadIdx.x, lane = tid & 63, l31 = lane & 31, half = lane >> 5;
  const int w = __builtin_amdgcn_readfirstlane(tid >> 6);
  const int L = p.L;

  {
    uint32_t* z = reinterpret_cast<uint32_t*>(&hl[0][0][0]);
    for (int i = tid; i < 2 * SQ * HROW / 2; i += 512) z[i] = 0u;
  }
  const int ubase = 32 * w + 4 * half;
  const int glane = ((d * 256 + 8 * w + half) * 32 + l31) * 16;
  const int clane = ((d * 64 + 8 * w + half) * 32 + l31) * 16;
  auto grs = [&](int t) { return mkrsrc(p.gates + (long long)(blockIdx.x * L + t) * (SQ * 2 * LG), SQ * 2 * LG * 4); };
  auto crs = [&](float* b, int t) { return mkrsrc(b + (long long)(blockIdx.x * L + t) * (SQ * 2 * LH), SQ * 2 * LH * 4); };
  auto xrs = [&](int t) { return mkrsrc(p.xn + (long long)(blockIdx.x * L + t) * (SQ * 128), SQ * 128 * 4); };
  auto hrs = [&](int t) { return mkrsrc(p.gates + (long long)(blockIdx.x * L + t) * (SQ * LG), SQ * 2 * LG * 2); };
  auto st_gate = [&](const f32x4& v, int t, int g, int j) {
    if constexpr (GF != 0) bst8(g == 2 ? enc_u16x4<true>(v) : enc_u16x4<false>(v), hrs(t), glane >> 1, (g * 64 + 2 * j) * 256);
    else bst(v, grs(t), glane, (g * 64 + 2 * j) * 512);
  };
  auto st_ch = [&](const f32x4& v, float* b, int t, int j) { bst(v, crs(b, t), clane, 2 * j * 512); };
  auto ld_x = [&](int t, int q) -> f32x4 { return bld(xrs(t), tid * 16, q * 8192); };
  auto st_x = [&](const f32x4& v, int buf, int q) {
    const int u = tid + 512 * q, quad = u >> 5, slot = u & 31;
    bf16x4 hi, lo;
    unpack_hl4(v, hi, lo);
    *reinterpret_cast<bf16x4*>(&xl[buf][0][slot * XROW + 4 * quad]) = hi;
    *reinterpret_cast<bf16x4*>(&xl[buf][1][slot * XROW + 4 * quad]) = lo;
  };

  float* cme = &cl[l31 * (LH + 4) + ubase];
#pragma unroll
  for (int j = 0; j < 4; ++j) *reinterpret_cast<f32x4*>(cme + 8 * j) = f32x4{0.f, 0.f, 0.f, 0.f};

  f32x4 bias[4][4];
#pragma unroll
  for (int g = 0; g < 4; ++g)
#pragma unroll
    for (int j = 0; j < 4; ++j)
      bias[g][j] = *reinterpret_cast<const f32x4*>(p.bias + d * LG + g * 256 + ubase + 8 * j) * (H16 ? 256.f : 1.f);

  const __amdgpu_buffer_rsrc_t wrs =
      F8 ? __builtin_amdgcn_make_buffer_rsrc(reinterpret_cast<unsigned char*>(const_cast<float*>(p.wpack)) +
                                                 (long long)(d * 8 + w) * F8_REGION, 0, F8_REGION, 0x00020000)
         : __builtin_amdgcn_make_buffer_rsrc(const_cast<float*>(p.wpack) + (long long)(d * 8 + w) * (FKS * 8 * 64 * 4), 0,
                                             FKS * 8 * 1024, 0x00020000);
  const int wlane = lane * 16;
  bf16x8 wr[2][8];
  auto refill = [&](int s, int kn, int zo) {
#pragma unroll
    for (int f = 0; f < 8; ++f) {
      if (F8 && kn >= 8) {
        if (f < 6) wr[s][f] = wload(wrs, wlane + f * 1024, zo + F8_HPART + (kn - 8) * F8_KSTEP);
      } else {
// ... 99 lines not shown
      for (int r = 0; r < 4; ++r) {
        const float ig = H16 ? c2_sig256(acc[0][4 * j + r]) : fsig(acc[0][4 * j + r]);
        const float fg = H16 ? c2_sig256(acc[1][4 * j + r]) : fsig(acc[1][4 * j + r]);
        const float gg = H16 ? c2_tanh256(acc[2][4 * j + r]) : ftanh(acc[2][4 * j + r]);
        const float og = H16 ? c2_sig256(acc[3][4 * j + r]) : fsig(acc[3][4 * j + r]);
        const float cn = fg * cold[r] + ig * gg;
        vi[r] = ig;
        vf[r] = fg;
        vg[r] = gg;
        vo[r] = og;
        vc[r] = cn;
        vh[r] = og * ftanh(cn);
      }
      bf16x4 h_hi, h_lo;
      split4(vh, h_hi, h_lo);
      if constexpr (H16) {
        *reinterpret_cast<u32x2*>(nhi + 8 * j) = enc_f16x4(vh);
        if constexpr (F8) {
          int c8 = 0;
          c8 = __builtin_amdgcn_cvt_pk_fp8_f32(vh[0], vh[1], c8, false);
          c8 = __builtin_amdgcn_cvt_pk_fp8_f32(vh[2], vh[3], c8, true);
          *reinterpret_cast<int*>(reinterpret_cast<unsigned char*>(&hl[cur ^ 1][1][0]) + l31 * H8ROW + ubase + 8 * j) = c8;
        }
      } else {
        *reinterpret_cast<bf16x4*>(nhi + 8 * j) = h_hi;
        *reinterpret_cast<bf16x4*>(nlo + 8 * j) = h_lo;
      }
      *reinterpret_cast<f32x4*>(cme + 8 * j) = vc;
      st_gate(vi, t, 0, j);
      st_gate(vf, t, 1, j);
      st_gate(vg, t, 2, j);
      st_gate(vo, t, 3, j);
      st_ch(vc, p.cbuf, t, j);
      st_ch(pack_hl4(h_hi, h_lo), p.hcat, t, j);
      __builtin_amdgcn_sched_barrier(0);
    }
    __syncthreads();
  }
}


struct fused64_lds {
  f32x4 xw[2][1024];
  __bf16 hl[2][2 * SQ * HROW];
  f32x4 c0l[8 * 2 * 4 * 32];
  float bs[LG];
};
template <int GF, bool W1 = false, bool H16 = false, bool F8 = false>
__device__ __forceinline__ void lstm_fwd_fused64_body(const ws_lstm_fused_args& p) {
  static_assert(!(W1 && H16), "W1 is a measurement build of the three-term kernel");
  static_assert(!F8 || H16, "the FP8 lo term belongs to the fp16-h kernel");
  __shared__ __attribute__((aligned(16))) fused64_lds sm;
  auto& xw = sm.xw;
  auto& hl = sm.hl;
  auto& c0l = sm.c0l;
  auto& bs = sm.bs;
  const int d = blockIdx.y;
  const int tid = threadIdx.x, lane = tid & 63, l31 = lane & 31, half = lane >> 5;
  const int w = __builtin_amdgcn_readfirstlane(tid >> 6);
  const int L = p.L;
  const int ntile = (p.nseq + SQ - 1) / SQ;
  const int tile0 = 2 * blockIdx.x;
  const unsigned live1 = tile0 + 1 < ntile ? 1u : 0u;

  {
    uint32_t* z = reinterpret_cast<uint32_t*>(&hl[0][0]);
    for (int i = tid; i < 2 * 2 * SQ * HROW / 2; i += 512) z[i] = 0u;
    for (int i = tid; i < LG; i += 512) bs[i] = (H16 ? 256.f : 1.f) * p.bias[d * LG + i];
  }
  const int ubase = 32 * w + 4 * half;
  const int glane = ((d * 256 + 8 * w + half) * 32 + l31) * 16;
  const int clane = ((d * 64 + 8 * w + half) * 32 + l31) * 16;
  auto blk = [&](int e, int t) { return (long long)((tile0 + e) * L + t); };
  auto lim = [&](int e, unsigned bytes) { return e == 0 ? bytes : bytes * live1; };
  auto grs = [&](int e, int t) { return mkrsrc(p.gates + blk(e, t) * (SQ * 2 * LG), lim(e, SQ * 2 * LG * 4)); };
  auto hrs = [&](int e, int t) { return mkrsrc(p.gates + blk(e, t) * (SQ * LG), lim(e, SQ * 2 * LG * 2)); };
  auto st_gate = [&](const f32x4& v, int e, int t, int g, int j) {
    if constexpr (GF != 0) bst8(g == 2 ? enc_u16x4<true>(v) : enc_u16x4<false>(v), hrs(e, t), glane >> 1, (g * 64 + 2 * j) * 256);
    else bst(v, grs(e, t), glane, (g * 64 + 2 * j) * 512);
  };
  auto crs = [&](float* b, int e, int t) { return mkrsrc(b + blk(e, t) * (SQ * 2 * LH), lim(e, SQ * 2 * LH * 4)); };
  auto xrs = [&](int e, int t) { return mkrsrc(p.xn + blk(e, t) * (SQ * 128), lim(e, SQ * 128 * 4)); };
  auto dma_x = [&](int e, int t) {
#pragma unroll
    for (int q = 0; q < 2; ++q)
      __builtin_amdgcn_raw_ptr_buffer_load_lds(xrs(e, t), (__attribute__((address_space(3))) void*)&xw[e][512 * q + 64 * w], 16,
                                               lane * 16, (512 * q + 64 * w) * 16, 0, WS_STREAM_AUX);
  };

  f32x4* c0 = &c0l[((w * 2 + half) * 4) * 32 + l31];
#pragma unroll
  for (int j = 0; j < 4; ++j) c0[32 * j] = f32x4{0.f, 0.f, 0.f, 0.f};
  f32x4 c1[4];
#pragma unroll
  for (int j = 0; j < 4; ++j) c1[j] = f32x4{0.f, 0.f, 0.f, 0.f};

  const __amdgpu_buffer_rsrc_t wrs =
      F8 ? __builtin_amdgcn_make_buffer_rsrc(reinterpret_cast<unsigned char*>(const_cast<float*>(p.wpack)) +
                                                 (long long)(d * 8 + w) * F8_REGION, 0, F8_REGION, 0x00020000)
         : __builtin_amdgcn_make_buffer_rsrc(const_cast<float*>(p.wpack) + (long long)(d * 8 + w) * (FKS * 8 * 64 * 4), 0,
                                             FKS * 8 * 1024, 0x00020000);
  const int wlane = lane * 16;
  bf16x8 wr[2][8];
  auto refill = [&](int s, int kn, int zo) {
#pragma unroll
    for (int f = 0; f < 8; ++f) {
      if (F8 && kn >= 8) {
        if (f < 6) wr[s][f] = wload(wrs, wlane + f * 1024, zo + F8_HPART + (kn - 8) * F8_KSTEP);
      } else if (!W1 || !(f & 1)) {
        wr[s][f] = wload(wrs, wlane + (f & 3) * 1024, zo + kn * 8192 + (f >> 2) * 4096);
      }
    }
  };
  refill(0, 0, 0);
  refill(1, 1, 0);
// ... 118 lines not shown
          const float gg = H16 ? c2_tanh256(acc[e][2][4 * j + r]) : ftanh(acc[e][2][4 * j + r]);
          const float og = H16 ? c2_sig256(acc[e][3][4 * j + r]) : fsig(acc[e][3][4 * j + r]);
          const float cn = fg * cold[r] + ig * gg;
          vi[r] = ig;
          vf[r] = fg;
          vg[r] = gg;
          vo[r] = og;
          vc[r] = cn;
          vh[r] = og * ftanh(cn);
        }
        bf16x4 h_hi, h_lo;
        split4(vh, h_hi, h_lo);
        if constexpr (H16) {
          *reinterpret_cast<u32x2*>(nhi + 8 * j) = enc_f16x4(vh);
          if constexpr (F8) {
            int c8 = 0;
            c8 = __builtin_amdgcn_cvt_pk_fp8_f32(vh[0], vh[1], c8, false);
            c8 = __builtin_amdgcn_cvt_pk_fp8_f32(vh[2], vh[3], c8, true);
            *reinterpret_cast<int*>(h8 + (32 * e + l31) * H8ROW + ubase + 8 * j) = c8;
          }
        } else {
          *reinterpret_cast<bf16x4*>(nhi + 8 * j) = h_hi;
          *reinterpret_cast<bf16x4*>(nlo + 8 * j) = h_lo;
        }
        if (e == 0)
          c0[32 * j] = vc;
        else
          c1[j] = vc;
        st_gate(vi, e, t, 0, j);
        st_gate(vf, e, t, 1, j);
        st_gate(vg, e, t, 2, j);
        st_gate(vo, e, t, 3, j);
        bst(vc, crs(p.cbuf, e, t), clane, 2 * j * 512);
        bst(pack_hl4(h_hi, h_lo), crs(p.hcat, e, t), clane, 2 * j * 512);
        __builtin_amdgcn_sched_barrier(0);
      }
    }
    if (p.hfmt & 2) asm volatile("s_waitcnt vmcnt(0)" ::: "memory");
    else asm volatile("s_waitcnt vmcnt(48)" ::: "memory");
    __syncthreads();
  }
}

__global__ __launch_bounds__(512, 1) void lstm_fwd_fused64_kernel(const ws_lstm_fused_args p) {
  lstm_fwd_fused64_body<0>(p);
}
__global__ __launch_bounds__(512, 1) void lstm_fwd_fused64h_kernel(const ws_lstm_fused_args p) {
  lstm_fwd_fused64_body<WS_GATES_H2>(p);
}
__global__ __launch_bounds__(512, 1) void lstm_fwd_fused64h_w1_kernel(const ws_lstm_fused_args p) {
  lstm_fwd_fused64_body<WS_GATES_H2, true>(p);
}
__global__ __launch_bounds__(512, 1) void lstm_fwd_fused64h16_kernel(const ws_lstm_fused_args p) {
  lstm_fwd_fused64_body<WS_GATES_H2, false, true>(p);
}
__global__ __launch_bounds__(512, 1) void lstm_fwd_fused64h8_kernel(const ws_lstm_fused_args p) {
  lstm_fwd_fused64_body<WS_GATES_H2, false, true, true>(p);
}

extern "C" int ws_lstm_fwd_fused(const ws_lstm_fused_args* a, void* stream) {
  WS_REQUIRE(a && a->gates && a->cbuf && a->hcat && a->xn && a->wpack && a->bias, "ws_lstm_fwd_fused: null pointer");
  WS_REQUIRE(a->nseq > 0 && a->L > 0, "ws_lstm_fwd_fused: bad nseq/L");
  WS_REQUIRE(a->gfmt >= WS_GATES_F32 && a->gfmt <= WS_GATES_H2F, "ws_lstm_fwd_fused: gfmt %d", a->gfmt);
  WS_REQUIRE((a->hfmt & ~7) == 0 && (!(a->hfmt & 1) || a->gfmt != WS_GATES_F32) && (!(a->hfmt & 4) || (a->hfmt & 1)),
             "ws_lstm_fwd_fused: hfmt %d (1 = fp16 h, pack from ws_lstm_pack_fused_h16; 5 = + FP8 lo term, pack from "
             "ws_lstm_pack_fused_h8; 2-byte gate formats only)", a->hfmt);
  const int ntile = (a->nseq + SQ - 1) / SQ;
  dim3 grid(ntile, 2), block(512);
  hipStream_t s = (hipStream_t)stream;
  const char* env = getenv("WS_FUSED_SEQS");
  static int cus = 0;
  if (!cus && hipDeviceGetAttribute(&cus, hipDeviceAttributeMultiprocessorCount, 0) != hipSuccess) cus = 256;
  const int rounds32 = (2 * ntile + cus - 1) / cus, rounds64 = (2 * ((ntile + 1) / 2) + cus - 1) / cus;
  const bool wide = env ? atoi(env) == 64 : 9 * rounds64 < 5 * rounds32;
  ws_prof_begin(WS_PROF_LSTM_FWD, s);
  const char* w1 = getenv("WS_FUSED_W1");
  if ((a->hfmt & 4) && wide)
    hipLaunchKernelGGL(lstm_fwd_fused64h8_kernel, dim3((ntile + 1) / 2, 2), block, 0, s, *a);
  else if (a->hfmt & 4)
    hipLaunchKernelGGL((lstm_fwd_fused_kernel<WS_GATES_H2, true, true>), grid, block, 0, s, *a);
  else if ((a->hfmt & 1) && wide)
    hipLaunchKernelGGL(lstm_fwd_fused64h16_kernel, dim3((ntile + 1) / 2, 2), block, 0, s, *a);
  else if (a->hfmt & 1)
    hipLaunchKernelGGL((lstm_fwd_fused_kernel<WS_GATES_H2, true>), grid, block, 0, s, *a);
  else if (wide && a->gfmt && w1 && atoi(w1) == 1)
    hipLaunchKernelGGL(lstm_fwd_fused64h_w1_kernel, dim3((ntile + 1) / 2, 2), block, 0, s, *a);
  else if (wide && a->gfmt)
    hipLaunchKernelGGL(lstm_fwd_fused64h_kernel, dim3((ntile + 1) / 2, 2), block, 0, s, *a);
  else if (wide)
    hipLaunchKernelGGL(lstm_fwd_fused64_kernel, dim3((ntile + 1) / 2, 2), block, 0, s, *a);
  else if (a->gfmt)
    hipLaunchKernelGGL(lstm_fwd_fused_kernel<WS_GATES_H2>, grid, block, 0, s, *a);
  else
    hipLaunchKernelGGL(lstm_fwd_fused_kernel<0>, grid, block, 0, s, *a);
  ws_prof_end(WS_PROF_LSTM_FWD, s);
  return ws_check_launch("ws_lstm_fwd_fused");
}
```

wesep_amd/dev.py:

```python
import ctypes as C
import os
from typing import NamedTuple, Optional

import numpy as np
import torch

from . import _lib as L

BIG = 1 << 30


def gemm_mode() -> str:
    return os.environ.get("WESEP_GEMM", "bf16x3")


def _mode_bit(mode):
    return 4 if (mode or gemm_mode()) == "bf16x3" else 0
GN_EPS = float(np.finfo(np.float32).eps)


class Rows(NamedTuple):
    div: int
    s1: int
    s2: int
# ... 324 lines not shown


def _bptt_bytes(gfmt: int) -> int:
    return {L.GATES_F32: 40, L.GATES_H2: 24, L.GATES_H2S: 32, L.GATES_H2F: 24}[gfmt]


def gates_fmt() -> int:
    return {"h2": L.GATES_H2F, "h2b": L.GATES_H2, "h2s": L.GATES_H2S, "f32": L.GATES_F32}[os.environ.get("WESEP_GATES", "h2")]


def blh_floats(nblocks: int, C_: int) -> int:
    return nblocks * 32 * C_ // 2


def _lstm_args(gates, cbuf, hcat, wpack, sm: SeqMap, mode, dhcat=None, run_if=None, gfmt=0, gates_in=None, dgates=None,
               amax=None, rfmt=0, dxn=None, wxpack=None):
    for n, t in (("gates", gates), ("cbuf", cbuf), ("hcat", hcat), ("wpack", wpack), ("dhcat", dhcat),
                 ("gates_in", gates_in), ("dgates", dgates), ("dxn", dxn), ("wxpack", wxpack)):
        _chk(t, n)
    a = L.LstmArgs()
    a.gates, a.cbuf, a.hcat, a.dhcat, a.wpack = _p(gates), _p(cbuf), _p(hcat), _p(dhcat), _p(wpack)
    a.sq_s1, a.sq_s2, a.step_rows = sm.s1, sm.s2, sm.step_rows
    a.nseq, a.sq_div, a.L, a.mode = sm.nseq, sm.div, sm.L, mode
    a.run_if = C.c_void_p(run_if.data_ptr()) if run_if is not None else None
    a.gates_in, a.dgates, a.gfmt, a.rfmt = _p(gates_in), _p(dgates), gfmt, rfmt
    a.amax = C.c_void_p(amax.data_ptr()) if amax is not None else None
    if dxn is not None:
        if dxn.dim() != 3 or dxn.shape[0] != 2 or dxn.shape[2] != 128 or getattr(sm, "nvalid", 0):
            raise L.WesepHipError(f"lstm_bwd: dxn must be [2, P, 128] on a sequence map without padding sequences, got {tuple(dxn.shape)}")
        a.dxn, a.dxn_dir_stride, a.wxpack = _p(dxn), dxn.shape[1] * 128, _p(wxpack)
    return a


def lstm_fwd(gates, cbuf, hcat, wpack, sm: SeqMap, mode=L.LSTM_BF16X3, run_if=None, gfmt=0, gates_in=None):
    a = _lstm_args(gates, cbuf, hcat, wpack, sm, mode, run_if=run_if, gfmt=gfmt, gates_in=gates_in)
    if run_if is None:
        u = ALG_LSTM_UNITS or L.LSTM_H
        _alg("lstm_fwd", sm.nseq * sm.L * 2 * u * (16 + (2 if gfmt else 4) * 4 + 8), 2 * sm.nseq * sm.L * 2 * 4 * u * u)
    L.check(L.lib().ws_lstm_fwd(C.byref(a), L.stream_ptr()), "ws_lstm_fwd")


def lstm_bwd(gates, cbuf, hcat, dhcat, wpack, sm: SeqMap, mode=L.LSTM_BF16X3, gfmt=0, dgates=None, run_if=None, amax=None,
             rfmt=0, dxn=None, wxpack=None):
    a = _lstm_args(gates, cbuf, hcat, wpack, sm, mode, dhcat, gfmt=gfmt, dgates=dgates, run_if=run_if, amax=amax, rfmt=rfmt,
                   dxn=dxn, wxpack=wxpack)
    if run_if is None:
        _alg("lstm_bwd", _bptt_bytes(gfmt) * sm.nseq * sm.L * 2 * (ALG_LSTM_UNITS or L.LSTM_H),
             2 * sm.nseq * sm.L * 2 * 4 * (ALG_LSTM_UNITS or L.LSTM_H) ** 2)
    L.check(L.lib().ws_lstm_bwd(C.byref(a), L.stream_ptr()), "ws_lstm_bwd")


_CU_COUNT = {}


def cu_count(device) -> int:
    key = (device.type, device.index)
    if key not in _CU_COUNT:
        _CU_COUNT[key] = torch.cuda.get_device_properties(device).multi_processor_count
    return _CU_COUNT[key]


def lstm_cluster_ok(sm: SeqMap, device) -> bool:
    if os.environ.get("WESEP_LSTM_CLUSTER", "1") == "0":
        return False
    return sm.nseq % 64 == 0 and (sm.nseq // 32) * 8 <= cu_count(device) and sm.L >= 64


class _ClusterScratch:

    def __init__(self, device):
        self.device = device
# ... 101 lines not shown
    sc = _cluster_scratch(gates.device)
    xchg, flags = sc.get(ncl * 2 * 8 * 8192 // 4, ncl * 8 + 8)
    a = L.LstmClusterArgs()
    a.gates, a.cbuf, a.hcat, a.whh_f, a.whh_r = _p(gates), _p(cbuf), _p(hcat), _p(whh_f), _p(whh_r)
    a.gfmt, a.gates_in = gfmt, _p(gates_in)
    a.xchg, a.flags = C.c_void_p(xchg.data_ptr()), C.c_void_p(flags.data_ptr())
    a.status = C.c_void_p((status if status is not None else sc.status).data_ptr())
    a.nseq, a.L, a.dbg = sm.nseq, sm.L, dbg
    u = ALG_LSTM_UNITS or L.LSTM_H
    _alg("lstm_fwd", sm.nseq * sm.L * 2 * u * (16 + (2 if gfmt else 4) * 4 + 8), 2 * sm.nseq * sm.L * 2 * 4 * u * u)
    L.check(L.lib().ws_lstm_fwd_cluster(C.byref(a), L.stream_ptr()), "ws_lstm_fwd_cluster")
    return flags[ncl * 8:ncl * 8 + 1]


_FALLBACK_SCRATCH = {}


def fallback_scratch(device, nfloats: int) -> torch.Tensor:
    key = (device.type, device.index, L.stream_ptr().value if device.type == "cuda" and torch.cuda.is_available() else 0)
    buf = _FALLBACK_SCRATCH.get(key)
    if buf is None or buf.numel() < nfloats:
        buf = _FALLBACK_SCRATCH[key] = torch.empty(nfloats, device=device, dtype=torch.float32)
    return buf[:nfloats]


def lstm_cluster2_on() -> bool:
    return os.environ.get("WESEP_LSTM_CLUSTER2", "1") != "0"


def cluster2_rfmt() -> int:
    return 1 if os.environ.get("WESEP_CLUSTER2_F8", "0") == "1" else 0


def lstm_fwd_cluster2(gates, cbuf, hcat, xn, wcat, bcat, whh_f, whh_r, sm: SeqMap, status=None, dbg=0, dbg_buf=None, rfmt=None):
    for n, t in (("gates", gates), ("cbuf", cbuf), ("hcat", hcat), ("xn", xn), ("wcat", wcat), ("bcat", bcat),
                 ("whh_f", whh_f), ("whh_r", whh_r)):
        _chk(t, n)
    ncl = sm.nseq // 32
    sc = _cluster_scratch(gates.device)
    xchg, flags = sc.get(ncl * 2 * 8 * 4096 // 4, ncl * 8 + 8)
    a = L.LstmCluster2Args()
    a.gates, a.cbuf, a.hcat, a.xn, a.wcat, a.bcat = _p(gates), _p(cbuf), _p(hcat), _p(xn), _p(wcat), _p(bcat)
    a.whh_f, a.whh_r = _p(whh_f), _p(whh_r)
    tw = flags[ncl * 8:ncl * 8 + 1]
    a.xchg, a.tword = C.c_void_p(xchg.data_ptr()), C.c_void_p(tw.data_ptr())
    a.status = C.c_void_p((status if status is not None else sc.status).data_ptr())
    a.nseq, a.L, a.dbg = sm.nseq, sm.L, dbg
    a.rfmt = cluster2_rfmt() if rfmt is None else rfmt
    a.dbg_buf = C.c_void_p(dbg_buf.data_ptr()) if dbg_buf is not None else None
    u = ALG_LSTM_UNITS or L.LSTM_H
    _alg("lstm_fwd", sm.nseq * sm.L * (2 * u * 16 + 4 * 128), 2 * sm.nseq * sm.L * 2 * 4 * u * (u + 128))
    L.check(L.lib().ws_lstm_fwd_cluster2(C.byref(a), L.stream_ptr()), "ws_lstm_fwd_cluster2")
    return tw


def lstm_bwd_cluster(gates, cbuf, dhcat, whh_f, whh_r, sm: SeqMap, status=None, dbg=0):
    for n, t in (("gates", gates), ("cbuf", cbuf), ("dhcat", dhcat), ("whh_f", whh_f), ("whh_r", whh_r)):
        _chk(t, n)
    ncl = sm.nseq // 32
    sc = _cluster_scratch(gates.device)
    xchg, flags = sc.get(ncl * 2 * 64 * 8192 // 4, ncl * 8 + 8)
    a = L.LstmClusterArgs()
    a.gates, a.cbuf, a.dhcat, a.whh_f, a.whh_r = _p(gates), _p(cbuf), _p(dhcat), _p(whh_f), _p(whh_r)
    a.xchg, a.flags = C.c_void_p(xchg.data_ptr()), C.c_void_p(flags.data_ptr())
    a.status = C.c_void_p(status.data_ptr() if status is not None else sc.status.data_ptr() + 4)
    a.nseq, a.L, a.dbg = sm.nseq, sm.L, dbg
    L.check(L.lib().ws_lstm_bwd_cluster(C.byref(a), L.stream_ptr()), "ws_lstm_bwd_cluster")
    return flags[ncl * 8:ncl * 8 + 1]


def lstm_pair_ok(sm: SeqMap, device) -> bool:
    if os.environ.get("WESEP_LSTM_PAIR_BWD", "1") == "0":
        return False
    return 4 * (-(-sm.nseq // 32)) <= cu_count(device) // 2 and sm.L >= 64


def lstm_pack_pair(whh_f, whh_r, pack, f16=False):
    for n, t in (("whh_f", whh_f), ("whh_r", whh_r), ("pack", pack)):
        _chk(t, n)
    fn = (L.lib().ws_lstm_pack_pair, L.lib().ws_lstm_pack_pair_f16, L.lib().ws_lstm_pack_pair_f8,
          L.lib().ws_lstm_pack_pair_f8mx)[int(f16)]
    L.check(fn(_p(whh_f), _p(whh_r), _p(pack), L.stream_ptr()), "ws_lstm_pack_pair")


# ... 281 lines not shown
        return
    L.check(L.lib().ws_gemm_p2b(C.byref(a), L.stream_ptr()), "ws_gemm_p2b")


def gemm_b2p(*, A, K: int, sm: SeqMap, Wpack, C_out, ldc: int, N=128, bias=None, R=None, a_fmt=0, amax=None, a16_out=None):
    for n, t in (("A", A), ("Wpack", Wpack), ("bias", bias), ("C", C_out), ("R", R), ("a16_out", a16_out)):
        _chk(t, n)
    if a16_out is not None and a_fmt != 0:
        raise L.WesepHipError("gemm_b2p: a16_out goes with a_fmt = 0 (split-pair A)")
    a = L.GemmB2PArgs()
    a.A, a.Wpack, a.bias, a.R, a.C = _p(A), _p(Wpack), _p(bias), _p(R), _p(C_out)
    a.sm = _smc(sm)
    a.ldc, a.N, a.K, a.a_fmt = ldc, N, K, a_fmt
    a.amax = C.c_void_p(amax.data_ptr()) if amax is not None else None
    a.a16_out = _p(a16_out)
    if ALG is not None:
        rows = (getattr(sm, "nvalid", 0) or sm.nseq) * sm.L
        _alg("gemm_nt", rows * ((2 if a_fmt else 4) * K + 4 * N * (1 + (R is not None)) + (2 * K if a16_out is not None else 0))
             + 4 * N * K, 2 * rows * N * K)
    L.check(L.lib().ws_gemm_b2p(C.byref(a), L.stream_ptr()), "ws_gemm_b2p")


def tnb_splits(nblk: int, gtiles: int):
    cap = int(os.environ.get("WESEP_TNB_MAXSPLIT", "64"))
    nsplit = max(1, min(cap, int(os.environ.get("WESEP_TNB_WGS", "256")) // gtiles, nblk))
    if nsplit >= 8:
        nsplit -= nsplit % 8
    bps = -(-nblk // nsplit)
    return nsplit, bps


def gemm_tnb(*, G, g_width: int, g_off: int, g_cols: int, A0, a0_width: int, a0_off: int, a0_cols: int,
             nblk: int, L_: int, slab, nsplit: int, blocks_per_split: int, a0_shift=0, A1=None, a1_width=0,
             a1_off=0, a1_cols=0, a1_shift=0, bslab=None, aslab=None, g_fmt=0, amax=None, a_fmt=0):
    for n, t in (("G", G), ("A0", A0), ("A1", A1), ("slab", slab), ("bslab", bslab), ("aslab", aslab)):
        _chk(t, n)
    a = L.GemmTNBArgs()
    a.G, a.A0, a.A1, a.slab, a.bslab, a.aslab = _p(G), _p(A0), _p(A1), _p(slab), _p(bslab), _p(aslab)
    a.slab_stride = g_cols * (a0_cols + a1_cols)
    a.bslab_stride = g_cols
    a.aslab_stride = a0_cols + a1_cols
    a.g_width, a.g_off, a.g_cols = g_width, g_off, g_cols
    a.a0_width, a.a0_off, a.a0_cols, a.a0_shift = a0_width, a0_off, a0_cols, a0_shift
    a.a1_width, a.a1_off, a.a1_cols, a.a1_shift = a1_width, a1_off, a1_cols, a1_shift
    a.nblk, a.L, a.nsplit, a.blocks_per_split, a.g_fmt, a.a_fmt = nblk, L_, nsplit, blocks_per_split, g_fmt, a_fmt
    a.amax = C.c_void_p(amax.data_ptr()) if amax is not None else None
    if ALG is not None:
        rows, acols = nblk * 32, a0_cols + a1_cols
        _alg("gemm_tn", rows * ((2 if g_fmt else 4) * g_cols + (2 if a_fmt else 4) * acols) + 4 * nsplit * g_cols * acols,
             2 * rows * g_cols * acols)
    L.check(L.lib().ws_gemm_tnb(C.byref(a), L.stream_ptr()), "ws_gemm_tnb")


LN_EPS = 1e-5


def _call(name, *args):
    L.check(getattr(L.lib(), name)(*args, L.stream_ptr()), name)


def flat_stats(x, ngroups: int, n_per_group: int, stats, eps=LN_EPS, nchunk=None):
    if nchunk is None:
        nchunk = max(1, min(max(1, 512 // ngroups), n_per_group // 16384))
    scratch = torch.empty(ngroups, nchunk, 4, device=x.device, dtype=torch.float32)
    for n, t in (("x", x), ("stats", stats)):
        _chk(t, n)
    _call("ws_flat_stats", _p(x), ngroups, n_per_group, eps, nchunk, _p(scratch), _p(stats))


def prelu_fwd(x, rb, a, rows: int, Cc: int, rows_per_r: int, y):
    for n, t in (("x", x), ("rb", rb), ("a", a), ("y", y)):
        _chk(t, n)
    _call("ws_prelu_fwd", _p(x), _p(rb), _p(a), rows, Cc, rows_per_r, _p(y))


def prelu_bwd(pre, dy, a, dx):
    for n, t in (("pre", pre), ("dy", dy), ("a", a), ("dx", dx)):
        _chk(t, n)
    n = pre.numel()
    nslab = max(1, min(1024, n // 4096))
    slab = torch.empty(nslab, device=pre.device, dtype=torch.float32)
    _call("ws_prelu_bwd", _p(pre), _p(dy), _p(a), n, _p(dx), _p(slab), nslab)
    da = torch.empty(1, device=pre.device, dtype=torch.float32)
# ... 160 lines not shown
    _chk(loss, "loss")
    _chk(dlogits, "dlogits")
    R, S = logits.shape
    _call("ws_cross_entropy", _p(logits), C.c_void_p(label.data_ptr()), R, S, _p(loss), _p(dlogits))


def lstm_fuse_ok(nseq: int, cluster: bool) -> bool:
    if os.environ.get("WESEP_LSTM_FUSE", "1") == "0" or cluster:
        return False
    return lstm_blk_mode(nseq) == L.LSTM_BF16X3_BLK


def lstm_fused_hfmt(gfmt) -> int:
    if gfmt == L.GATES_F32 or os.environ.get("WESEP_FUSED_H16", "1") == "0":
        return 0
    return 5 if os.environ.get("WESEP_FUSED_F8", "1") != "0" else 1


def lstm_pack_fused(wih_f, wih_r, whh_f, whh_r, pack, hfmt=0):
    for n, t in (("wih_f", wih_f), ("wih_r", wih_r), ("whh_f", whh_f), ("whh_r", whh_r), ("pack", pack)):
        _chk(t, n)
    _call("ws_lstm_pack_fused_h8" if hfmt & 4 else "ws_lstm_pack_fused_h16" if hfmt & 1 else "ws_lstm_pack_fused",
          _p(wih_f), _p(wih_r), _p(whh_f), _p(whh_r), _p(pack))


def lstm_fwd_fused(gates, cbuf, hcat, xn, wpack, bias, sm: SeqMap, gfmt=0, hfmt=0):
    for n, t in (("gates", gates), ("cbuf", cbuf), ("hcat", hcat), ("xn", xn), ("wpack", wpack), ("bias", bias)):
        _chk(t, n)
    a = L.LstmFusedArgs()
    a.gates, a.cbuf, a.hcat, a.xn, a.wpack, a.bias = _p(gates), _p(cbuf), _p(hcat), _p(xn), _p(wpack), _p(bias)
    a.nseq, a.L, a.gfmt = sm.nseq, sm.L, gfmt
    a.hfmt = hfmt | (2 if os.environ.get("WESEP_FUSED_DRAIN", "0") == "1" else 0)
    u = ALG_LSTM_UNITS or L.LSTM_H
    _alg("lstm_fwd", sm.nseq * sm.L * (2 * u * ((2 if gfmt else 4) * 4 + 8) + 4 * 128), 2 * sm.nseq * sm.L * 2 * 4 * u * (u + 128))
    L.check(L.lib().ws_lstm_fwd_fused(C.byref(a), L.stream_ptr()), "ws_lstm_fwd_fused")


def conv_out(n: int, k: int, s: int, p: int) -> int:
    return (n + 2 * p - k) // s + 1


def im2col(x, R: int, H: int, W: int, Cc: int, k: int, s: int, p: int, patches, ldp: int):
    _chk(x, "x")
    _chk(patches, "patches")
    _call("ws_im2col", _p(x), R, H, W, Cc, k, s, p, ldp, _p(patches))


def col2im(dpatches, R: int, H: int, W: int, Cc: int, k: int, s: int, p: int, dx):
    _chk(dpatches, "dpatches")
    _chk(dx, "dx")
    _call("ws_col2im", _p(dpatches), R, H, W, Cc, k, s, p, _p(dx))


def tstp_fwd(x, R: int, F: int, T: int, Cc: int, stats, eps=1e-7):
    _chk(x, "x")
    _chk(stats, "stats")
    _call("ws_tstp_fwd", _p(x), R, F, T, Cc, eps, _p(stats))


def tstp_bwd(x, stats, dstats, R: int, F: int, T: int, Cc: int, dx):
    for n, t in (("x", x), ("stats", stats), ("dstats", dstats), ("dx", dx)):
        _chk(t, n)
    _call("ws_tstp_bwd", _p(x), _p(stats), _p(dstats), R, F, T, Cc, _p(dx))


def mhastp_sizes(R: int, T: int, Q: int, H: int, layers: int, ds: int, dm: int):
    blk, work = C.c_longlong(0), C.c_longlong(0)
# ... 610 lines not shown
```

wesep_amd/functional.py:

```python
import os

import numpy as np
import torch

from . import _lib as L
from . import dev
from .dev import BIG, Geom, Rows, SeqMap, StatMap, flat
from .blstm_core import (G4, H, PAIR_STAMPS, PackCache, WeightPacks, WGradBox, WGradCarrierFn, _NO_CACHE,
                         _PROBE_SAT, _cluster_dbg, _empty, _h2_probe, _pair_dbg, _pending, _probe_round, _reduce_new,
                         _side_stream, amax_word, band_dx, band_rfmt, blstm_bptt, blstm_dxn, blstm_forward,
                         blstm_weight_grads, consume_once, defer_wgrad, dxn_fmt, flush_deferred_wgrads, keep_for_side,
                         make_plan, mark_wgrads_ready, pair_rfmt, tnb_a16, weight_grads, wgrad_hold, zero_words)

NBIN = 257
HOP = 128


def _need_cuda(t, who):
    if not t.is_cuda:
        raise L.WesepHipError(f"{who}: wesep_amd has no CPU path; move the model and inputs to the GPU")


def _view_maps(view, R, K, Tf, N):
    if view == "time":
# ... 136 lines not shown
        dev.group_stats(z, geo, stats)
    cache = cache if cache is not None else _NO_CACHE
    sig = cache.begin(wparams)
    plan = make_plan(seq, d, grad, gn_geo=geo, ragged=ragged) if ragged else make_plan(seq, d, grad, gn_geo=geo)
    W = WeightPacks(cache, sig, plan.lmode, plan.pair_rfmt, *wparams[:9])
    steps = dict(steps=(frames, K)) if ragged else {}
    out, saved = blstm_forward(plan, W, z, seq, res=z, bias=proj_b,
                               norm=dict(stats=stats, gamma=norm_w, beta=norm_b, stat_map=smap), **steps)
    return out, stats, plan, W, saved


class ResRNNBlkFn(torch.autograd.Function):

    @staticmethod
    def forward(ctx, z, dummy, box, cache, view, norm_w, norm_b, wih_f, whh_f, bih_f, bhh_f, wih_r, whh_r, bih_r,
                bhh_r, proj_w, proj_b):
        z = z.contiguous()
        d = z.device
        out, stats, plan, W, saved = _resrnn_blk_fwd(
            z, view, norm_w, norm_b, (wih_f, whh_f, bih_f, bhh_f, wih_r, whh_r, bih_r, bhh_r, proj_w, proj_b), cache,
            any(ctx.needs_input_grad))
        ctx.save_for_backward(z, stats, norm_w, *saved)
        if view == "time" and box is not None and plan.grad:
            key = (d.type, d.index)
            _TIME_LEFT[key] = _TIME_LEFT.get(key, 0) + 1
        ctx.view, ctx.box, ctx.plan, ctx.packs = view, box, plan, W
        ctx.consumed = False
        return out

    @staticmethod
    def backward(ctx, dout):
        consume_once(ctx, "ResRNN")
        z, stats, norm_w, gates, cbuf, hcat, xn, hcat16 = ctx.saved_tensors
        plan, W, box = ctx.plan, ctx.packs, ctx.box
        dout = dout.contiguous()
        R, K, Tf, N = z.shape
        P = R * K * Tf
        d = z.device
        geo, smap, seq, _ = _view_maps(ctx.view, R, K, Tf, N)
        dg, dout_bl, amax, dxn2 = blstm_bptt(plan, W, gates, cbuf, hcat, dout, seq, release=ctx.view == "time")
        wg = blstm_weight_grads(plan, dg, xn, hcat, dout_bl, amax, hcat16, seq, box)
        del dout_bl
        if box is not None and ctx.view == "time":
            key = (d.type, d.index)
            _TIME_LEFT[key] = _TIME_LEFT.get(key, 1) - 1
            if _TIME_LEFT[key] <= 0 and tail_flush():
                flush_deferred_wgrads(d)
        dxn, dxn_r = blstm_dxn(plan, W, dg, amax, dxn2, seq, P)
        dz = torch.empty_like(z)
        dgb = _empty(d, 2, N)
        if dev.gn_bwd_fused_ok(geo):
            ns2 = min(1024, -(-geo.ngroups // 4))
            pslab = _empty(d, ns2 + dev.tree_groups(ns2), 2, N)
            dev.gn_bwd_fused(z, dxn, stats, geo, norm_w, dz, ns2, pslab, res=dout, pout=dgb,
                             counter=zero_words(d, 1 + dev.tree_groups(ns2)), dxn2=dxn_r)
        elif dev.gn_bwd_apply_pg_ok(geo):
            ab = _empty(d, geo.ngroups, 2)
            dev.gn_bwd_reduce(z, dxn, stats, geo, ab, gamma=norm_w)
            pslab = _empty(d, geo.ngroups + dev.tree_groups(geo.ngroups), 2, N)
            dev.gn_bwd_apply_pg(z, dxn, stats, ab, geo, dz, norm_w, pslab, dgb, zero_words(d, 1 + dev.tree_groups(geo.ngroups)),
                                res=dout)
        else:
            ab = _empty(d, geo.ngroups, 2)
            dev.gn_bwd_reduce(z, dxn, stats, geo, ab, gamma=norm_w)
            ns2 = min(1024, geo.ngroups)
            pslab = _empty(d, ns2, 2, N)
# ... 545 lines not shown
```

wesep_amd/functional_tfgridnet.py:

```python
import numpy as np
import os

import torch

from . import _lib as L
from . import dev
from .dev import BIG, Rows, SeqMap, flat
from .blstm_core import PackCache, WeightPacks, blstm_bptt, blstm_dxn, blstm_forward, blstm_weight_grads, consume_once, make_plan
from .functional import _empty, _need_cuda, _reduce_new
from .functional_tasnet import _cln_geom, _gemm, _transposed, _wgrad, norm_backward

HP = L.LSTM_H
G4P = 4 * HP


def pad_lstm(w_ih, w_hh, b_ih, b_hh, col_perm=None):
    h = w_hh.shape[1]
    if h > HP:
        raise NotImplementedError(f"TF-GridNet lstm_hidden_units={h} > {HP}")
    d = w_ih.device
    rows = (torch.arange(4, device=d).unsqueeze(1) * HP + torch.arange(h, device=d).unsqueeze(0)).reshape(-1)
    wi = w_ih if col_perm is None else w_ih[:, col_perm]
    wi_p = torch.zeros(G4P, wi.shape[1], device=d, dtype=torch.float32).index_copy(0, rows, wi)
    wh_c = torch.zeros(4 * h, HP, device=d, dtype=torch.float32)
# ... 360 lines not shown
class BlstmLinearBlkFn(torch.autograd.Function):

    @staticmethod
    def forward(ctx, y, res, geo, dummy, box, wih_f, wih_r, b_f, b_r, whf, whr, lin_w, lin_b):
        _need_cuda(y, "TF-GridNet")
        nseq, Lr = geo[:2]
        strided = geo[2:] if len(geo) > 2 else None
        d = y.device
        pad = 0
        if Lr >= 64 and nseq % 64 and (-(-nseq // 64) * 64 // 32) * 8 <= dev.cu_count(d):
            pad = -(-nseq // 64) * 64 - nseq
        ns = nseq + pad
        if pad and strided is None:
            z = torch.zeros(pad * Lr, 128, device=d, dtype=torch.float32)
            y, res = torch.cat([y, z], 0), torch.cat([res, z], 0)
        y, res = y.contiguous(), res.contiguous()
        seq = SeqMap(ns, BIG, 0, Lr, 1, Lr) if strided is None else SeqMap(ns, *strided, Lr, nvalid=nseq)
        plan = make_plan(seq, d, any(ctx.needs_input_grad))
        zero = torch.zeros(G4P, device=d, dtype=torch.float32)
        cache = PackCache()
        sig = cache.begin((wih_f, whf, b_f, wih_r, whr, b_r, lin_w))
        W = WeightPacks(cache, sig, plan.lmode, plan.pair_rfmt, wih_f, whf, b_f.contiguous(), zero, wih_r, whr,
                          b_r.contiguous(), zero, lin_w)
        out, saved = blstm_forward(plan, W, y, seq, res=res, bias=lin_b.contiguous())
        ctx.save_for_backward(*saved)
        ctx.geo, ctx.seq, ctx.plan, ctx.packs, ctx.box = (nseq, Lr, ns), seq, plan, W, box
        ctx.consumed = False
        return out[:nseq * Lr] if (pad and strided is None) else out

    @staticmethod
    def backward(ctx, dout):
        consume_once(ctx, "TF-GridNet BLSTM")
        gates, cbuf, hcat, xn, hcat16 = ctx.saved_tensors
        nseq, Lr, ns = ctx.geo
        seq, plan, W, box = ctx.seq, ctx.plan, ctx.packs, ctx.box
        d = dout.device
        dout = dout.contiguous()
        dres = dout
        appended = ns != nseq and not seq.nvalid
        if appended:
            dout = torch.cat([dout, torch.zeros((ns - nseq) * Lr, 128, device=d, dtype=torch.float32)], 0)
        dg, dout_bl, amax, dxn2 = blstm_bptt(plan, W, gates, cbuf, hcat, dout, seq, release=plan.bptt in ("pair", "cluster"))
        wg = blstm_weight_grads(plan, dg, xn, hcat, dout_bl, amax, hcat16, seq, box, order=(0, 4, 2, 6, 1, 5, 8, 9))
        del dout_bl
        dy, _ = blstm_dxn(plan, W, dg, amax, dxn2, seq, (ns if appended else nseq) * Lr)
        if appended:
            dy = dy[:nseq * Lr]
        gd = torch.zeros((), device=d) if box is not None else None
        return (dy, dres, None, gd, None) + tuple(wg)
```

Measured before the change: 341.2 utterances/s.

## Use fp16 hcat for projection weight-gradient GEMM and optionally store only fp16 hcat

Adds an fp16-G variant of the split-pair TN GEMM (ws_gemm_htnb) that reads the fp16 hcat copy and splits it into bf16 hi/lo pairs in registers. With the default flag on, the projection weight gradient uses it, so the fp32 hcat no longer has to be saved for backward. A second, opt-in path (WESEP_H16_ONLY) has the LSTM forward kernels write hcat only as fp16 and feeds it into an fp16/FP8 projection GEMM. Together these cut hcat memory traffic and the size of saved activations. The cost is lower precision of h in the weight gradients and extra conversion work inside the GEMM kernel.

```diff
diff --git a/include/wesep_hip.h b/include/wesep_hip.h
--- a/include/wesep_hip.h
+++ b/include/wesep_hip.h
@@ -292,6 +292,7 @@
   int a_fmt, pad_;
 } ws_gemm_tnb_args;
 int ws_gemm_tnb(const ws_gemm_tnb_args* a, void* stream);
+int ws_gemm_htnb(const ws_gemm_tnb_args* a, void* stream);
 
 typedef struct ws_bands {
   const int* band_of_bin;
diff --git a/wesep_amd/_lib.py b/wesep_amd/_lib.py
--- a/wesep_amd/_lib.py
+++ b/wesep_amd/_lib.py
@@ -192,6 +192,7 @@
     "ws_gemm_p2b_len": (_i, [C.POINTER(GemmP2BArgs), _p, _i, _p]),
     "ws_gemm_b2p": (_i, [C.POINTER(GemmB2PArgs), _p]),
     "ws_gemm_tnb": (_i, [C.POINTER(GemmTNBArgs), _p]),
+    "ws_gemm_htnb": (_i, [C.POINTER(GemmTNBArgs), _p]),
     "ws_stft_bandsplit": (_i, [_p, _i, _i, C.POINTER(Bands), _p, _p]),
     "ws_stft_bandsplit_len": (_i, [_p, _i, _i, _p, C.POINTER(Bands), _p, _p]),
     "ws_mask_istft_frames": (_i, [_p, _p, _i, _i, C.POINTER(Bands), _p, _p]),
diff --git a/wesep_amd/blstm_core.py b/wesep_amd/blstm_core.py
--- a/wesep_amd/blstm_core.py
+++ b/wesep_amd/blstm_core.py
@@ -57,6 +57,18 @@
 
 def dxn_fmt(g_fmt) -> int:
     return 3 if g_fmt == 2 and os.environ.get("WESEP_DXN_F8", "1") != "0" else g_fmt
+
+
+def dwp16() -> bool:
+    return os.environ.get("WESEP_DWP16", "1") != "0"
+
+
+def h16_only() -> bool:
+    return os.environ.get("WESEP_H16_ONLY", "0") == "1"
+
+
+def proj_fmt() -> int:
+    return 3 if os.environ.get("WESEP_PROJ_F8", "1") != "0" else 2
 
 
 def band_rfmt(gfmt, lmode) -> int:
@@ -329,6 +341,10 @@
             out = _empty(d, N * 2 * H)
             dev.pack_w(W("pw"), N, 2 * H, 2 * H, out, order=1)
             return out
+        if kind in ("proj16", "proj8"):
+            out = _empty(d, N * 2 * H)
+            dev.pack_w(W("pw"), N, 2 * H, 2 * H, out, order=1, f16=1 if kind == "proj16" else 2)
+            return out
         if kind == "projT":
             out = _empty(d, 2 * H * N)
             dev.pack_w(W("pw"), 2 * H, N, 2 * H, out, trans=True, order=0)
@@ -350,12 +366,18 @@
     band_rfmt: int
     band_dx: bool
     a_fmt: int
+    h16: bool = False
+    p_fmt: int = 0
+    dwp16: bool = False
+
+
+_PROJ_KIND = {0: "proj", 2: "proj16", 3: "proj8"}
 
 
 _WIHT_KIND = {0: "wihT", 1: "wihT", 2: "wihT16", 3: "wihT8"}
 
 
-def make_plan(seq, device, grad, gn_geo=None, ragged=False) -> BlstmPlan:
+def make_plan(seq, device, grad, gn_geo=None, ragged=False, on_gpu=None) -> BlstmPlan:
     lmode = dev.lstm_blk_mode(seq.nseq)
     cluster = dev.lstm_cluster_ok(seq, device)
     bptt = _bptt_kind(seq, device, cluster)
@@ -371,10 +393,15 @@
         fwd = "stream"
     g_fmt = {L.GATES_H2: 1, L.GATES_H2F: 2}.get(gfmt, 0)
     brf = band_rfmt(gfmt, lmode) if grad and bptt == "stream" else 0
+    a16 = gfmt == L.GATES_H2F and grad and tnb_a16()
+    on_dev = device.type == "cuda" if on_gpu is None else bool(on_gpu)
+    h16 = (a16 and h16_only() and on_dev and
+           (fwd in ("cluster2", "stream") or (fwd == "fused" and dev.lstm_fused_hfmt(gfmt) & 1)))
     return BlstmPlan(
         nb=dev.bl_num_blocks(seq), lmode=lmode, cluster=cluster, fwd=fwd, bptt=bptt, grad=grad, gfmt=gfmt, g_fmt=g_fmt,
-        a16=gfmt == L.GATES_H2F and grad and tnb_a16(), pair_rfmt=pair_rfmt(gfmt) if grad and bptt == "pair" else 0,
-        band_rfmt=brf, band_dx=bool(brf) and gn_geo is not None and band_dx(brf, seq, gn_geo), a_fmt=dxn_fmt(g_fmt))
+        a16=a16, pair_rfmt=pair_rfmt(gfmt) if grad and bptt == "pair" else 0,
+        band_rfmt=brf, band_dx=bool(brf) and gn_geo is not None and band_dx(brf, seq, gn_geo), a_fmt=dxn_fmt(g_fmt),
+        h16=h16, p_fmt=proj_fmt() if h16 else 0, dwp16=h16 or (a16 and dwp16() and on_dev))
 
 
 def consume_once(ctx, who):
@@ -396,21 +423,25 @@
     wcat, bcat = W("cat")
     whf, whr = W("whh")
     xn = _empty(d, nb, 32 * N)
-    cbuf, hcat = _empty(d, nb, 32 * 2 * H), _empty(d, nb, 32 * 2 * H)
+    h16 = plan.h16
+    cbuf = _empty(d, nb, 32 * 2 * H)
+    hcat = None if h16 else _empty(d, nb, 32 * 2 * H)
     gates = _empty(d, dev.blh_floats(nb, 2 * G4)) if h2 else _empty(d, nb, 32 * 2 * G4)
     xn16 = _empty(d, dev.blh_floats(nb, N)) if plan.a16 else None
     hcat16 = _empty(d, dev.blh_floats(nb, 2 * H)) if plan.a16 else None
+    hout = hcat16 if h16 else hcat
+    h16kw = dict(h16=True) if h16 else {}
     if plan.fwd == "fused":
         dev.gemm_p2b(A=x, lda=N, sm=seq, Wpack=None, N=0, C_out=None, A_bl=xn, A_bl16=xn16, **norm)
         hf = dev.lstm_fused_hfmt(gfmt)
-        dev.lstm_fwd_fused(gates, cbuf, hcat, xn, W("fused8" if hf & 4 else "fused16" if hf else "fused"), bcat, seq, gfmt=gfmt,
-                           hfmt=hf)
+        dev.lstm_fwd_fused(gates, cbuf, hout, xn, W("fused8" if hf & 4 else "fused16" if hf else "fused"), bcat, seq, gfmt=gfmt,
+                           hfmt=hf | (8 if h16 else 0))
     elif plan.fwd == "cluster2":
         dev.gemm_p2b(A=x, lda=N, sm=seq, Wpack=None, N=0, C_out=None, A_bl=xn, A_bl16=xn16, **norm)
-        tw = dev.lstm_fwd_cluster2(gates, cbuf, hcat, xn, wcat, bcat, whf, whr, seq, dbg=_cluster_dbg())
+        tw = dev.lstm_fwd_cluster2(gates, cbuf, hout, xn, wcat, bcat, whf, whr, seq, dbg=_cluster_dbg(), **h16kw)
         pre = dev.fallback_scratch(d, nb * 32 * 2 * G4)
         dev.gemm_p2b(A=x, lda=N, sm=seq, Wpack=W("wih"), N=2 * G4, C_out=pre, bias=bcat, run_if=tw, **norm)
-        dev.lstm_fwd(gates, cbuf, hcat, W("hh")[0], seq, lmode, run_if=tw, gfmt=gfmt, gates_in=pre)
+        dev.lstm_fwd(gates, cbuf, hout, W("hh")[0], seq, lmode, run_if=tw, gfmt=gfmt, gates_in=pre, **h16kw)
         del pre
     else:
         pre = _empty(d, nb, 32 * 2 * G4) if h2 else gates
@@ -425,10 +456,14 @@
                 dev.gemm_p2b(run_if=tw, **xproj)
             dev.lstm_fwd(gates, cbuf, hcat, W("hh")[0], seq, lmode, run_if=tw, **rec)
         else:
-            dev.lstm_fwd(gates, cbuf, hcat, W("hh")[0], seq, lmode, **rec)
+            dev.lstm_fwd(gates, cbuf, hout, W("hh")[0], seq, lmode, **rec, **h16kw)
         del pre
     out = torch.empty_like(res)
-    dev.gemm_b2p(A=hcat, K=2 * H, sm=seq, Wpack=W("proj"), C_out=out, ldc=N, bias=bias, R=res, a16_out=hcat16)
+    if h16:
+        dev.gemm_b2p(A=hcat16, K=2 * H, sm=seq, Wpack=W(_PROJ_KIND[plan.p_fmt]), C_out=out, ldc=N, bias=bias, R=res,
+                     a_fmt=plan.p_fmt, amax=amax_word(d))
+    else:
+        dev.gemm_b2p(A=hcat, K=2 * H, sm=seq, Wpack=W("proj"), C_out=out, ldc=N, bias=bias, R=res, a16_out=hcat16)
     if _h2_probe() and not h2:
         if _h2_probe() & 1:
             _probe_round(gates, "f16")
@@ -448,7 +483,7 @@
             W("hh8")
             if plan.band_dx:
                 W("wx8")
-    return out, (gates, cbuf, hcat, xn16 if plan.a16 else xn, hcat16)
+    return out, (gates, cbuf, None if plan.dwp16 else hcat, xn16 if plan.a16 else xn, hcat16)
 
 
 def blstm_bptt(plan, W, gates, cbuf, hcat, dout, seq, release):
@@ -498,7 +533,7 @@
     return dg, dout_bl, amax, dxn2
 
 
-def weight_grads(gates, xn, hcat, dout_bl, seq, nb, g_fmt=0, amax=None, hcat16=None):
+def weight_grads(gates, xn, hcat, dout_bl, seq, nb, g_fmt=0, amax=None, hcat16=None, h16=False):
     d = gates.device
     a_fmt = 1 if hcat16 is not None else 0
     if _h2_probe() & 192 and not torch.cuda.is_available() and not a_fmt:
@@ -513,8 +548,8 @@
         dout_bl = (dout_bl * S).half().float() / S
     ns, bps = dev.tnb_splits(nb, (2 * H) // 128)
     slab, aslab = _empty(d, ns, 2 * H * N), _empty(d, ns, N)
-    dev.gemm_tnb(G=hcat, g_width=2 * H, g_off=0, g_cols=2 * H, A0=dout_bl, a0_width=N, a0_off=0, a0_cols=N,
-                 nblk=nb, L_=seq.L, slab=slab, nsplit=ns, blocks_per_split=bps, aslab=aslab)
+    dev.gemm_tnb(G=hcat16 if h16 else hcat, g_width=2 * H, g_off=0, g_cols=2 * H, A0=dout_bl, a0_width=N, a0_off=0, a0_cols=N,
+                 nblk=nb, L_=seq.L, slab=slab, nsplit=ns, blocks_per_split=bps, aslab=aslab, **(dict(g16=True) if h16 else {}))
     dproj_w = _reduce_new(slab, ns, 2 * H * N, (2 * H, N)).t().contiguous()
     dproj_b = _reduce_new(aslab, ns, N, (N,))
     ns, bps = dev.tnb_splits(nb, G4 // 128)
@@ -535,12 +570,12 @@
 
 def blstm_weight_grads(plan, dg, xn, hcat, dout_bl, amax, hcat16, seq, box, order=tuple(range(10))):
     if box is None:
-        wg = weight_grads(dg, xn, hcat, dout_bl, seq, plan.nb, plan.g_fmt, amax, hcat16)
+        wg = weight_grads(dg, xn, hcat, dout_bl, seq, plan.nb, plan.g_fmt, amax, hcat16, plan.dwp16)
         return [wg[i] for i in order]
     prod = torch.cuda.current_stream()
 
     def job(side):
-        wg = weight_grads(dg, xn, hcat, dout_bl, seq, plan.nb, plan.g_fmt, amax, hcat16)
+        wg = weight_grads(dg, xn, hcat, dout_bl, seq, plan.nb, plan.g_fmt, amax, hcat16, plan.dwp16)
         box.grads = [wg[i] for i in order]
         box.event = torch.cuda.Event()
         box.event.record(side)
diff --git a/wesep_amd/csrc/gemm_blk.hip b/wesep_amd/csrc/gemm_blk.hip
--- a/wesep_amd/csrc/gemm_blk.hip
+++ b/wesep_amd/csrc/gemm_blk.hip
@@ -541,8 +541,9 @@
 
 typedef __bf16 bf16x2 __attribute__((ext_vector_type(2)));
 
-template <int TA, bool ASUM>
+template <int TA, bool ASUM, bool GH = false>
 __global__ __launch_bounds__(512, 2) void gemm_tnb_kernel(const ws_gemm_tnb_args p) {
+  static_assert(!GH || TA == 1, "fp16 G of the split-pair kernel: one A tile (thread = G group or A group)");
   constexpr int NCOL = 128 * (1 + TA);
   constexpr int PLANE = NCOL * TB_LD;
   constexpr int NG = (1 + TA) / 2;
@@ -566,8 +567,8 @@
     const int part = g >> 8, quad = (g >> 3) & 31, sg = g & 7;
     gcol[r] = part * 128 + 4 * quad;
     if (part == 0) {
-      gbase[r] = p.G + (long long)((p.g_off + gt * 128) / 4 + quad) * 128 + sg * 16;
-      gstride[r] = 32LL * p.g_width;
+      gbase[r] = p.G + (long long)((p.g_off + gt * 128) / 4 + quad) * (GH ? 64 : 128) + sg * (GH ? 8 : 16);
+      gstride[r] = (GH ? 16LL : 32LL) * p.g_width;
       gshift[r] = 0;
     } else {
       const int c0 = (part - 1) * 128;
@@ -580,6 +581,7 @@
     }
   }
   const int sg = tid & 7;
+  const bool gthread = GH && w < 4;
 
   f32x4 rq[2][NG][4];
   bool use[2][NG];
@@ -591,7 +593,8 @@
       use[slot][r] = sa >= 0 && sa < L;
       const float* src = gbase[r] + (long long)(use[slot][r] ? b + gshift[r] : b) * gstride[r];
 #pragma unroll
-      for (int j = 0; j < 4; ++j) rq[slot][r][j] = *reinterpret_cast<const f32x4*>(src + 4 * j);
+      for (int j = 0; j < 4; ++j)
+        if (j < 2 || !gthread) rq[slot][r][j] = *reinterpret_cast<const f32x4*>(src + 4 * j);
     }
   };
   float csum[NG][4];
@@ -602,10 +605,21 @@
   auto store_piece = [&](int slot, __bf16* lds, unsigned live, int pc) {
     const int r = pc >> 2, c = pc & 3;
     unsigned e[4];
-#pragma unroll
-    for (int j = 0; j < 4; ++j) {
-      const float f = rq[slot][r][j][c];
-      e[j] = __float_as_uint(f);
+    if (gthread) {
+#pragma unroll
+      for (int j = 0; j < 4; ++j) {
+        const float wf = rq[slot][r][j >> 1][2 * (j & 1) + (c >> 1)];
+        const unsigned wd = __float_as_uint(wf);
+        const float x = (float)__builtin_bit_cast(_Float16, (unsigned short)((c & 1) ? wd >> 16 : wd & 0xffffu));
+        const __bf16 hi = (__bf16)x, lo = (__bf16)(x - (float)hi);
+        e[j] = ((unsigned)__builtin_bit_cast(unsigned short, hi) << 16) | (unsigned)__builtin_bit_cast(unsigned short, lo);
+      }
+    } else {
+#pragma unroll
+      for (int j = 0; j < 4; ++j) {
+        const float f = rq[slot][r][j][c];
+        e[j] = __float_as_uint(f);
+      }
     }
     if (r > 0) {
       const unsigned m = use[slot][r] ? 0xffffffffu : 0u;
@@ -1023,6 +1037,26 @@
         if (first) p.aslab[(long long)split * p.aslab_stride + acol[r] - 128 + c] = t;
       }
   }
+}
+
+extern "C" int ws_gemm_htnb(const ws_gemm_tnb_args* a, void* stream) {
+  WS_REQUIRE(a && a->G && a->A0 && a->slab, "ws_gemm_htnb: null pointer");
+  WS_REQUIRE(a->g_cols > 0 && a->g_cols % 128 == 0 && a->g_off % 4 == 0 && a->g_width % 4 == 0 && a->g_off + a->g_cols <= a->g_width,
+             "ws_gemm_htnb: G column range");
+  WS_REQUIRE(a->a0_cols == 128 && a->a0_off % 4 == 0 && a->a0_width % 4 == 0 && a->a0_off + 128 <= a->a0_width && a->a1_cols == 0 &&
+                 a->a0_shift == 0,
+             "ws_gemm_htnb: A is 128 unshifted columns of A0 (a0_cols = %d, a1_cols = %d, a0_shift = %d)", a->a0_cols, a->a1_cols,
+             a->a0_shift);
+  WS_REQUIRE(a->g_fmt == 0 && a->a_fmt == 0, "ws_gemm_htnb: g_fmt / a_fmt must be 0 (G is unscaled fp16 by definition, A holds BLS pairs)");
+  WS_REQUIRE(a->nblk > 0 && a->L > 0 && a->nblk % a->L == 0 && a->nsplit > 0 && a->blocks_per_split > 0 &&
+                 (long long)a->nsplit * a->blocks_per_split >= a->nblk,
+             "ws_gemm_htnb: bad block split");
+  hipStream_t s = (hipStream_t)stream;
+  dim3 grid(a->nsplit, a->g_cols / 128), block(512);
+  ws_prof_begin(WS_PROF_GEMM_TN, s);
+  hipLaunchKernelGGL((gemm_tnb_kernel<1, true, true>), grid, block, 0, s, *a);
+  ws_prof_end(WS_PROF_GEMM_TN, s);
+  return ws_check_launch("ws_gemm_htnb");
 }
 
 extern "C" int ws_gemm_tnb(const ws_gemm_tnb_args* a, void* stream) {
diff --git a/wesep_amd/csrc/lstm.hip b/wesep_amd/csrc/lstm.hip
--- a/wesep_amd/csrc/lstm.hip
+++ b/wesep_amd/csrc/lstm.hip
@@ -372,9 +372,12 @@
              a->gfmt);
   WS_REQUIRE(a->gfmt != WS_GATES_H2S || !bwd || a->dgates, "%s: WS_GATES_H2S needs dgates", who);
   WS_REQUIRE(a->gfmt == WS_GATES_F32 || ((a->mode >> 8) & 7) == 0, "%s: probe builds are WS_GATES_F32 only", who);
-  WS_REQUIRE(a->rfmt == 0 || ((a->rfmt == 2 || a->rfmt == 3) && bwd && a->mode == WS_LSTM_BF16X3_BLK && a->gfmt == WS_GATES_H2F),
+  WS_REQUIRE(a->rfmt == 0 || ((a->rfmt == 2 || a->rfmt == 3) && bwd && a->mode == WS_LSTM_BF16X3_BLK && a->gfmt == WS_GATES_H2F) ||
+                 (a->rfmt == 1 && !bwd && (a->mode == WS_LSTM_BF16X3_BLK || a->mode == WS_LSTM_BF16X3_BLK16) &&
+                  a->gfmt != WS_GATES_F32),
              "%s: rfmt %d (2 / 3 = fp16 recurrence on fp16 + FP8 weights, 3: the lo term on the FP8 MFMA: ws_lstm_bwd, "
-             "WS_LSTM_BF16X3_BLK, WS_GATES_H2F only)", who, a->rfmt);
+             "WS_LSTM_BF16X3_BLK, WS_GATES_H2F only; 1 = hcat leaves as fp16 in BLH: ws_lstm_fwd, blocked-layout modes with a "
+             "2-byte gate format only)", who, a->rfmt);
   WS_REQUIRE(!a->dxn || (bwd && a->rfmt == 2 && a->wxpack && a->dxn_dir_stride > 0 && a->dxn_dir_stride < (1ll << 29) && !a->run_if),
              "%s: dxn (d(xn) inside the BPTT, ABI v19) needs rfmt 2, wxpack (ws_lstm_pack_dx_f8), 0 < dxn_dir_stride < 2^29 floats "
              "(32-bit store offsets) and no run_if", who);
diff --git a/wesep_amd/csrc/lstm_bf16.hip b/wesep_amd/csrc/lstm_bf16.hip
--- a/wesep_amd/csrc/lstm_bf16.hip
+++ b/wesep_amd/csrc/lstm_bf16.hip
@@ -138,7 +138,7 @@
   return 0;
 }
 
-template <bool BLK, int DBG, int GF = 0>
+template <bool BLK, int DBG, int GF = 0, bool HS = false>
 __global__ __launch_bounds__(512, 2) void lstm_fwd_bf16_kernel(const ws_lstm_args p) {
   __shared__ __attribute__((aligned(16))) __bf16 hl[2][2][SQ * HROW];
   __shared__ __attribute__((aligned(16))) float cl[SQ * (LH + 4)];
@@ -181,6 +181,8 @@
     if constexpr (BLK) bst(v, crs(b, t), clane, 2 * j * 512);
     else *reinterpret_cast<f32x4*>(b + coff(t, j)) = v;
   };
+  static_assert(!HS || (BLK && GF != 0), "fp16 hcat: blocked layout, 2-byte gate formats");
+  auto h16rs = [&](int t) { return mkrsrc(p.hcat + (long long)(blockIdx.x * L + t) * (SQ * LH), SQ * 2 * LH * 2); };
 
   float* cme = &cl[l31 * (LH + 4) + ubase];
 #pragma unroll
@@ -290,8 +292,12 @@
         st_gate(vg, t, 2, j);
         st_gate(vo, t, 3, j);
         st_ch(vc, p.cbuf, t, j);
-        if constexpr (BLK) st_ch(pack_hl4(h_hi, h_lo), p.hcat, t, j);
-        else st_ch(vh, p.hcat, t, j);
+        if constexpr (BLK) {
+          if constexpr (HS) bst8(enc_h16_pair(h_hi, h_lo), h16rs(t), clane >> 1, 2 * j * 256);
+          else st_ch(pack_hl4(h_hi, h_lo), p.hcat, t, j);
+        } else {
+          st_ch(vh, p.hcat, t, j);
+        }
       }
       __builtin_amdgcn_sched_barrier(0);
     }
@@ -627,6 +633,10 @@
 
 int ws_launch_lstm_fwd_bf16(const ws_lstm_args* a, hipStream_t s) {
   dim3 grid((a->nseq + SQ - 1) / SQ, 2), block(512);
+  if (a->rfmt == 1) {
+    hipLaunchKernelGGL((lstm_fwd_bf16_kernel<true, 0, WS_GATES_H2F, true>), grid, block, 0, s, *a);
+    return 0;
+  }
   WS_DBG_DISPATCH(lstm_fwd_bf16_kernel)
   return 0;
 }
diff --git a/wesep_amd/csrc/lstm_bf16_common.h b/wesep_amd/csrc/lstm_bf16_common.h
--- a/wesep_amd/csrc/lstm_bf16_common.h
+++ b/wesep_amd/csrc/lstm_bf16_common.h
@@ -121,6 +121,17 @@
   for (int j = 0; j < 4; ++j) h[j] = (_Float16)vs[j];
   return __builtin_bit_cast(u32x2, h);
 }
+__device__ __forceinline__ u32x2 enc_h16_pair(const bf16x4& hi, const bf16x4& lo) {
+  const u32x2 hb = __builtin_bit_cast(u32x2, hi), lb = __builtin_bit_cast(u32x2, lo);
+  f16x4 h;
+#pragma unroll
+  for (int j = 0; j < 4; ++j) {
+    const unsigned hw = (j & 1) ? (hb[j >> 1] & 0xffff0000u) : (hb[j >> 1] << 16);
+    const unsigned lw = (j & 1) ? (lb[j >> 1] & 0xffff0000u) : (lb[j >> 1] << 16);
+    h[j] = (_Float16)(__uint_as_float(hw) + __uint_as_float(lw));
+  }
+  return __builtin_bit_cast(u32x2, h);
+}
 template <int GF>
 __device__ __forceinline__ u32x2 enc_dgates(const f32x4& v, const bf16x4& hi) {
   if constexpr (GF == WS_GATES_H2F) return enc_f16x4(v);
diff --git a/wesep_amd/csrc/lstm_bf16_s16.hip b/wesep_amd/csrc/lstm_bf16_s16.hip
--- a/wesep_amd/csrc/lstm_bf16_s16.hip
+++ b/wesep_amd/csrc/lstm_bf16_s16.hip
@@ -54,7 +54,7 @@
   return 0;
 }
 
-template <int GF>
+template <int GF, bool HS = false>
 __global__ __launch_bounds__(512, 2) void lstm_fwd_s16_kernel(const ws_lstm_args p) {
   __shared__ __attribute__((aligned(16))) __bf16 hl[2][2][S16 * HROW];
   __shared__ __attribute__((aligned(16))) float cl[S16 * (LH + 4)];
@@ -80,6 +80,7 @@
     else bst(v, grs(t), glane, (g * 64 + 4 * tu) * 512);
   };
   auto st_ch = [&](const f32x4& v, float* b, int t, int tu) { bst(v, crs(b, t), clane, 4 * tu * 512); };
+  auto h16rs = [&](int t) { return mkrsrc(p.hcat + (long long)(tile * L + t) * (SQ * LH), SQ * 2 * LH * 2); };
 
   const int ubase = 32 * w + 4 * mq;
   float* cme = &cl[n * (LH + 4) + ubase];
@@ -186,7 +187,8 @@
       st_gate(vg, t, 2, tu);
       st_gate(vo, t, 3, tu);
       st_ch(vc, p.cbuf, t, tu);
-      st_ch(pack_hl4(h_hi, h_lo), p.hcat, t, tu);
+      if constexpr (HS) bst8(enc_h16_pair(h_hi, h_lo), h16rs(t), clane >> 1, 4 * tu * 256);
+      else st_ch(pack_hl4(h_hi, h_lo), p.hcat, t, tu);
       __builtin_amdgcn_sched_barrier(0);
     }
     __syncthreads();
@@ -342,7 +344,8 @@
 
 int ws_launch_lstm_fwd_s16(const ws_lstm_args* a, hipStream_t s) {
   dim3 grid(2 * ((a->nseq + SQ - 1) / SQ), 2), block(512);
-  if (a->gfmt) hipLaunchKernelGGL(lstm_fwd_s16_kernel<WS_GATES_H2>, grid, block, 0, s, *a);
+  if (a->gfmt && a->rfmt == 1) hipLaunchKernelGGL((lstm_fwd_s16_kernel<WS_GATES_H2, true>), grid, block, 0, s, *a);
+  else if (a->gfmt) hipLaunchKernelGGL(lstm_fwd_s16_kernel<WS_GATES_H2>, grid, block, 0, s, *a);
   else hipLaunchKernelGGL(lstm_fwd_s16_kernel<0>, grid, block, 0, s, *a);
   return 0;
 }
diff --git a/wesep_amd/csrc/lstm_cluster2.hip b/wesep_amd/csrc/lstm_cluster2.hip
--- a/wesep_amd/csrc/lstm_cluster2.hip
+++ b/wesep_amd/csrc/lstm_cluster2.hip
@@ -142,6 +142,8 @@
   const int gts = (int)(L * gblk * 4), cts = (int)(L * cblk * 4);
   auto hrs = [&](int t) { return mkrsrc(p.gates + ((long long)2 * cc * L + t) * (gblk / 2), 0x7fffffffu); };
   auto crs = [&](float* b, int t) { return mkrsrc(b + ((long long)2 * cc * L + t) * cblk, 0x7fffffffu); };
+  const bool h16s = (p.rfmt & 2) != 0;
+  auto h16rs = [&](int t) { return mkrsrc(p.hcat + ((long long)2 * cc * L + t) * (cblk / 2), 0x7fffffffu); };
   const char* xbase = reinterpret_cast<const char*>(p.xn);
   auto xld = [&](int t, int q) -> f32x4 {
     const long long blk = (long long)(2 * cc + st) * L + t;
@@ -196,7 +198,12 @@
         bst8(u32x2{pr[2], pr[3]}, hrs(tprev), (gvo + e * gts) >> 1, (2 * g2 + 1) * 64 * 256);
       }
       bst(e == 0 ? c4 : outc[mt], crs(p.cbuf, tprev), cvo + e * cts, 0);
-      bst(outl[2][ct], crs(p.hcat, tprev), cvo + e * cts, 0);
+      if (h16s) {
+        const u32x4 hp = __builtin_bit_cast(u32x4, outl[2][ct]);
+        bst8(u32x2{hp[0], hp[1]}, h16rs(tprev), (cvo + e * cts) >> 1, 0);
+      } else {
+        bst(outl[2][ct], crs(p.hcat, tprev), cvo + e * cts, 0);
+      }
     }
   };
 
@@ -264,7 +271,12 @@
       if (!xrole) outc[mt] = c4;
       bf16x4 hi, lo;
       split4(vh, hi, lo);
-      outl[2][tid] = pack_hl4(hi, lo);
+      if (h16s) {
+        const u32x2 h2 = enc_h16_pair(hi, lo);
+        outl[2][tid] = __builtin_bit_cast(f32x4, u32x4{h2[0], h2[1], 0u, 0u});
+      } else {
+        outl[2][tid] = pack_hl4(hi, lo);
+      }
     }
     C2TS(3);
     xpart();
@@ -326,8 +338,9 @@
   e = hipMemsetAsync(a->tword, 0, sizeof(unsigned), s);
   WS_REQUIRE(e == hipSuccess, "ws_lstm_fwd_cluster2: hipMemsetAsync failed");
   ws_prof_begin(WS_PROF_LSTM_FWD, s);
-  WS_REQUIRE(a->rfmt == 0 || a->rfmt == 1, "ws_lstm_fwd_cluster2: rfmt %d (0: fp16 hi / lo of W_hh; 1: the lo term on the FP8 MFMA)", a->rfmt);
-  if (a->rfmt == 1) {
+  WS_REQUIRE(a->rfmt >= 0 && a->rfmt <= 3,
+             "ws_lstm_fwd_cluster2: rfmt %d (bit 0: the lo term of W_hh on the FP8 MFMA; bit 1: hcat leaves as fp16 in BLH)", a->rfmt);
+  if (a->rfmt & 1) {
     if (a->dbg & 2048) hipLaunchKernelGGL((lstm_fwd_cluster2_kernel<false, true, true>), dim3(grid), dim3(512), 0, s, *a);
     else if (a->dbg & 8) hipLaunchKernelGGL((lstm_fwd_cluster2_kernel<true, false, true>), dim3(grid), dim3(512), 0, s, *a);
     else hipLaunchKernelGGL((lstm_fwd_cluster2_kernel<false, false, true>), dim3(grid), dim3(512), 0, s, *a);
diff --git a/wesep_amd/csrc/lstm_fused.hip b/wesep_amd/csrc/lstm_fused.hip
--- a/wesep_amd/csrc/lstm_fused.hip
+++ b/wesep_amd/csrc/lstm_fused.hip
@@ -131,9 +131,10 @@
   return ws_check_launch("ws_lstm_pack_fused_h8");
 }
 
-template <int GF, bool H16 = false, bool F8 = false>
+template <int GF, bool H16 = false, bool F8 = false, bool HS = false>
 __global__ __launch_bounds__(512, 1) void lstm_fwd_fused_kernel(const ws_lstm_fused_args p) {
   static_assert(!F8 || H16, "the FP8 lo term belongs to the fp16-h kernel");
+  static_assert(!HS || H16, "fp16 hcat is built for the fp16-h kernels");
   __shared__ __attribute__((aligned(16))) __bf16 hl[2][2][SQ * HROW];
   __shared__ __attribute__((aligned(16))) __bf16 xl[2][2][SQ * XROW];
   __shared__ __attribute__((aligned(16))) float cl[SQ * (LH + 4)];
@@ -158,6 +159,11 @@
     else bst(v, grs(t), glane, (g * 64 + 2 * j) * 512);
   };
   auto st_ch = [&](const f32x4& v, float* b, int t, int j) { bst(v, crs(b, t), clane, 2 * j * 512); };
+  auto h16rs = [&](int t) { return mkrsrc(p.hcat + (long long)(blockIdx.x * L + t) * (SQ * LH), SQ * 2 * LH * 2); };
+  auto st_h = [&](const bf16x4& hi, const bf16x4& lo, int t, int j) {
+    if constexpr (HS) bst8(enc_h16_pair(hi, lo), h16rs(t), clane >> 1, 2 * j * 256);
+    else st_ch(pack_hl4(hi, lo), p.hcat, t, j);
+  };
   auto ld_x = [&](int t, int q) -> f32x4 { return bld(xrs(t), tid * 16, q * 8192); };
   auto st_x = [&](const f32x4& v, int buf, int q) {
     const int u = tid + 512 * q, quad = u >> 5, slot = u & 31;
@@ -323,7 +329,7 @@
       st_gate(vg, t, 2, j);
       st_gate(vo, t, 3, j);
       st_ch(vc, p.cbuf, t, j);
-      st_ch(pack_hl4(h_hi, h_lo), p.hcat, t, j);
+      st_h(h_hi, h_lo, t, j);
       __builtin_amdgcn_sched_barrier(0);
     }
     __syncthreads();
@@ -337,9 +343,10 @@
   f32x4 c0l[8 * 2 * 4 * 32];
   float bs[LG];
 };
-template <int GF, bool W1 = false, bool H16 = false, bool F8 = false>
+template <int GF, bool W1 = false, bool H16 = false, bool F8 = false, bool HS = false>
 __device__ __forceinline__ void lstm_fwd_fused64_body(const ws_lstm_fused_args& p) {
   static_assert(!(W1 && H16), "W1 is a measurement build of the three-term kernel");
+  static_assert(!HS || H16, "fp16 hcat is built for the fp16-h kernels");
   static_assert(!F8 || H16, "the FP8 lo term belongs to the fp16-h kernel");
   __shared__ __attribute__((aligned(16))) fused64_lds sm;
   auto& xw = sm.xw;
@@ -372,6 +379,7 @@
   };
   auto crs = [&](float* b, int e, int t) { return mkrsrc(b + blk(e, t) * (SQ * 2 * LH), lim(e, SQ * 2 * LH * 4)); };
   auto xrs = [&](int e, int t) { return mkrsrc(p.xn + blk(e, t) * (SQ * 128), lim(e, SQ * 128 * 4)); };
+  auto h16rs = [&](int e, int t) { return mkrsrc(p.hcat + blk(e, t) * (SQ * LH), lim(e, SQ * 2 * LH * 2)); };
   auto dma_x = [&](int e, int t) {
 #pragma unroll
     for (int q = 0; q < 2; ++q)
@@ -556,7 +564,8 @@
         st_gate(vg, e, t, 2, j);
         st_gate(vo, e, t, 3, j);
         bst(vc, crs(p.cbuf, e, t), clane, 2 * j * 512);
-        bst(pack_hl4(h_hi, h_lo), crs(p.hcat, e, t), clane, 2 * j * 512);
+        if constexpr (HS) bst8(enc_h16_pair(h_hi, h_lo), h16rs(e, t), clane >> 1, 2 * j * 256);
+        else bst(pack_hl4(h_hi, h_lo), crs(p.hcat, e, t), clane, 2 * j * 512);
         __builtin_amdgcn_sched_barrier(0);
       }
     }
@@ -580,15 +589,23 @@
 }
 __global__ __launch_bounds__(512, 1) void lstm_fwd_fused64h8_kernel(const ws_lstm_fused_args p) {
   lstm_fwd_fused64_body<WS_GATES_H2, false, true, true>(p);
+}
+
+__global__ __launch_bounds__(512, 1) void lstm_fwd_fused64h16s_kernel(const ws_lstm_fused_args p) {
+  lstm_fwd_fused64_body<WS_GATES_H2, false, true, false, true>(p);
+}
+__global__ __launch_bounds__(512, 1) void lstm_fwd_fused64h8s_kernel(const ws_lstm_fused_args p) {
+  lstm_fwd_fused64_body<WS_GATES_H2, false, true, true, true>(p);
 }
 
 extern "C" int ws_lstm_fwd_fused(const ws_lstm_fused_args* a, void* stream) {
   WS_REQUIRE(a && a->gates && a->cbuf && a->hcat && a->xn && a->wpack && a->bias, "ws_lstm_fwd_fused: null pointer");
   WS_REQUIRE(a->nseq > 0 && a->L > 0, "ws_lstm_fwd_fused: bad nseq/L");
   WS_REQUIRE(a->gfmt >= WS_GATES_F32 && a->gfmt <= WS_GATES_H2F, "ws_lstm_fwd_fused: gfmt %d", a->gfmt);
-  WS_REQUIRE((a->hfmt & ~7) == 0 && (!(a->hfmt & 1) || a->gfmt != WS_GATES_F32) && (!(a->hfmt & 4) || (a->hfmt & 1)),
+  WS_REQUIRE((a->hfmt & ~15) == 0 && (!(a->hfmt & 1) || a->gfmt != WS_GATES_F32) && (!(a->hfmt & 4) || (a->hfmt & 1)) &&
+                 (!(a->hfmt & 8) || (a->hfmt & 1)),
              "ws_lstm_fwd_fused: hfmt %d (1 = fp16 h, pack from ws_lstm_pack_fused_h16; 5 = + FP8 lo term, pack from "
-             "ws_lstm_pack_fused_h8; 2-byte gate formats only)", a->hfmt);
+             "ws_lstm_pack_fused_h8; bit 3, with bit 0 = hcat leaves as fp16 in BLH; 2-byte gate formats only)", a->hfmt);
   const int ntile = (a->nseq + SQ - 1) / SQ;
   dim3 grid(ntile, 2), block(512);
   hipStream_t s = (hipStream_t)stream;
@@ -599,7 +616,15 @@
   const bool wide = env ? atoi(env) == 64 : 9 * rounds64 < 5 * rounds32;
   ws_prof_begin(WS_PROF_LSTM_FWD, s);
   const char* w1 = getenv("WS_FUSED_W1");
-  if ((a->hfmt & 4) && wide)
+  if ((a->hfmt & 8) && (a->hfmt & 4) && wide)
+    hipLaunchKernelGGL(lstm_fwd_fused64h8s_kernel, dim3((ntile + 1) / 2, 2), block, 0, s, *a);
+  else if ((a->hfmt & 8) && (a->hfmt & 4))
+    hipLaunchKernelGGL((lstm_fwd_fused_kernel<WS_GATES_H2, true, true, true>), grid, block, 0, s, *a);
+  else if ((a->hfmt & 8) && wide)
+    hipLaunchKernelGGL(lstm_fwd_fused64h16s_kernel, dim3((ntile + 1) / 2, 2), block, 0, s, *a);
+  else if (a->hfmt & 8)
+    hipLaunchKernelGGL((lstm_fwd_fused_kernel<WS_GATES_H2, true, false, true>), grid, block, 0, s, *a);
+  else if ((a->hfmt & 4) && wide)
     hipLaunchKernelGGL(lstm_fwd_fused64h8_kernel, dim3((ntile + 1) / 2, 2), block, 0, s, *a);
   else if (a->hfmt & 4)
     hipLaunchKernelGGL((lstm_fwd_fused_kernel<WS_GATES_H2, true, true>), grid, block, 0, s, *a);
diff --git a/wesep_amd/dev.py b/wesep_amd/dev.py
--- a/wesep_amd/dev.py
+++ b/wesep_amd/dev.py
@@ -380,11 +380,11 @@
     return a
 
 
-def lstm_fwd(gates, cbuf, hcat, wpack, sm: SeqMap, mode=L.LSTM_BF16X3, run_if=None, gfmt=0, gates_in=None):
-    a = _lstm_args(gates, cbuf, hcat, wpack, sm, mode, run_if=run_if, gfmt=gfmt, gates_in=gates_in)
+def lstm_fwd(gates, cbuf, hcat, wpack, sm: SeqMap, mode=L.LSTM_BF16X3, run_if=None, gfmt=0, gates_in=None, h16=False):
+    a = _lstm_args(gates, cbuf, hcat, wpack, sm, mode, run_if=run_if, gfmt=gfmt, gates_in=gates_in, rfmt=1 if h16 else 0)
     if run_if is None:
         u = ALG_LSTM_UNITS or L.LSTM_H
-        _alg("lstm_fwd", sm.nseq * sm.L * 2 * u * (16 + (2 if gfmt else 4) * 4 + 8), 2 * sm.nseq * sm.L * 2 * 4 * u * u)
+        _alg("lstm_fwd", sm.nseq * sm.L * 2 * u * (16 + (2 if gfmt else 4) * 4 + (6 if h16 else 8)), 2 * sm.nseq * sm.L * 2 * 4 * u * u)
     L.check(L.lib().ws_lstm_fwd(C.byref(a), L.stream_ptr()), "ws_lstm_fwd")
 
 
@@ -552,7 +552,8 @@
     return 1 if os.environ.get("WESEP_CLUSTER2_F8", "0") == "1" else 0
 
 
-def lstm_fwd_cluster2(gates, cbuf, hcat, xn, wcat, bcat, whh_f, whh_r, sm: SeqMap, status=None, dbg=0, dbg_buf=None, rfmt=None):
+def lstm_fwd_cluster2(gates, cbuf, hcat, xn, wcat, bcat, whh_f, whh_r, sm: SeqMap, status=None, dbg=0, dbg_buf=None, rfmt=None,
+                      h16=False):
     for n, t in (("gates", gates), ("cbuf", cbuf), ("hcat", hcat), ("xn", xn), ("wcat", wcat), ("bcat", bcat),
                  ("whh_f", whh_f), ("whh_r", whh_r)):
         _chk(t, n)
@@ -566,10 +567,10 @@
     a.xchg, a.tword = C.c_void_p(xchg.data_ptr()), C.c_void_p(tw.data_ptr())
     a.status = C.c_void_p((status if status is not None else sc.status).data_ptr())
     a.nseq, a.L, a.dbg = sm.nseq, sm.L, dbg
-    a.rfmt = cluster2_rfmt() if rfmt is None else rfmt
+    a.rfmt = (cluster2_rfmt() if rfmt is None else rfmt) | (2 if h16 else 0)
     a.dbg_buf = C.c_void_p(dbg_buf.data_ptr()) if dbg_buf is not None else None
     u = ALG_LSTM_UNITS or L.LSTM_H
-    _alg("lstm_fwd", sm.nseq * sm.L * (2 * u * 16 + 4 * 128), 2 * sm.nseq * sm.L * 2 * 4 * u * (u + 128))
+    _alg("lstm_fwd", sm.nseq * sm.L * (2 * u * (14 if h16 else 16) + 4 * 128), 2 * sm.nseq * sm.L * 2 * 4 * u * (u + 128))
     L.check(L.lib().ws_lstm_fwd_cluster2(C.byref(a), L.stream_ptr()), "ws_lstm_fwd_cluster2")
     return tw
 
@@ -917,7 +918,7 @@
 
 def gemm_tnb(*, G, g_width: int, g_off: int, g_cols: int, A0, a0_width: int, a0_off: int, a0_cols: int,
              nblk: int, L_: int, slab, nsplit: int, blocks_per_split: int, a0_shift=0, A1=None, a1_width=0,
-             a1_off=0, a1_cols=0, a1_shift=0, bslab=None, aslab=None, g_fmt=0, amax=None, a_fmt=0):
+             a1_off=0, a1_cols=0, a1_shift=0, bslab=None, aslab=None, g_fmt=0, amax=None, a_fmt=0, g16=False):
     for n, t in (("G", G), ("A0", A0), ("A1", A1), ("slab", slab), ("bslab", bslab), ("aslab", aslab)):
         _chk(t, n)
     a = L.GemmTNBArgs()
@@ -932,8 +933,11 @@
     a.amax = C.c_void_p(amax.data_ptr()) if amax is not None else None
     if ALG is not None:
         rows, acols = nblk * 32, a0_cols + a1_cols
-        _alg("gemm_tn", rows * ((2 if g_fmt else 4) * g_cols + (2 if a_fmt else 4) * acols) + 4 * nsplit * g_cols * acols,
+        _alg("gemm_tn", rows * ((2 if g_fmt or g16 else 4) * g_cols + (2 if a_fmt else 4) * acols) + 4 * nsplit * g_cols * acols,
              2 * rows * g_cols * acols)
+    if g16:
+        L.check(L.lib().ws_gemm_htnb(C.byref(a), L.stream_ptr()), "ws_gemm_htnb")
+        return
     L.check(L.lib().ws_gemm_tnb(C.byref(a), L.stream_ptr()), "ws_gemm_tnb")
 
 
@@ -1160,7 +1164,8 @@
     a.nseq, a.L, a.gfmt = sm.nseq, sm.L, gfmt
     a.hfmt = hfmt | (2 if os.environ.get("WESEP_FUSED_DRAIN", "0") == "1" else 0)
     u = ALG_LSTM_UNITS or L.LSTM_H
-    _alg("lstm_fwd", sm.nseq * sm.L * (2 * u * ((2 if gfmt else 4) * 4 + 8) + 4 * 128), 2 * sm.nseq * sm.L * 2 * 4 * u * (u + 128))
+    _alg("lstm_fwd", sm.nseq * sm.L * (2 * u * ((2 if gfmt else 4) * 4 + (6 if hfmt & 8 else 8)) + 4 * 128),
+         2 * sm.nseq * sm.L * 2 * 4 * u * (u + 128))
     L.check(L.lib().ws_lstm_fwd_fused(C.byref(a), L.stream_ptr()), "ws_lstm_fwd_fused")
 
 
diff --git a/wesep_amd/functional.py b/wesep_amd/functional.py
--- a/wesep_amd/functional.py
+++ b/wesep_amd/functional.py
@@ -192,6 +192,7 @@
     def backward(ctx, dout):
         consume_once(ctx, "ResRNN")
         z, stats, norm_w, gates, cbuf, hcat, xn, hcat16 = ctx.saved_tensors
+        hcat = hcat if hcat is not None else hcat16
         plan, W, box = ctx.plan, ctx.packs, ctx.box
         dout = dout.contiguous()
         R, K, Tf, N = z.shape
diff --git a/wesep_amd/functional_tfgridnet.py b/wesep_amd/functional_tfgridnet.py
--- a/wesep_amd/functional_tfgridnet.py
+++ b/wesep_amd/functional_tfgridnet.py
@@ -416,6 +416,7 @@
     def backward(ctx, dout):
         consume_once(ctx, "TF-GridNet BLSTM")
         gates, cbuf, hcat, xn, hcat16 = ctx.saved_tensors
+        hcat = hcat if hcat is not None else hcat16
         nseq, Lr, ns = ctx.geo
         seq, plan, W, box = ctx.seq, ctx.plan, ctx.packs, ctx.box
         d = dout.device
```

Result: no change. 343.5 utterances/s, median of 6 (+0.7%).
